# kije/gpu_raytracer

Hardware: AMD Instinct MI355X
Metric: Mrays/s (higher is better)
Workload: dtype f32

## Files before the change

gpu_raytracer_amd/api.py:

```python
import ctypes as C
import os
import sys

import numpy as np

from . import types as T

_HERE = os.path.dirname(os.path.abspath(__file__))
LIB_PATH = os.environ.get("RT_HIP_LIB", os.path.join(_HERE, "librt_hip.so"))

RT_OK = 0
ERRORS = {-1: "RT_ERR_BAD_ARG", -2: "RT_ERR_OOM", -3: "RT_ERR_HIP", -4: "RT_ERR_NOT_UPLOADED", -5: "RT_ERR_INTERNAL"}
MODE_LEGACY, MODE_WAVEFRONT, MODE_EXTENDED = 0, 1, 2
FLAG_COUNTERS = 1
FLAG_NO_SHADOWS = 2
FLAG_KERNEL_V1 = 4
FLAG_KERNEL_SM = 8
FLAG_NO_SHADOW_GRID = 16
FLAG_KERNEL_PIPELINE = 32
FLAG_NO_BEAMS = 64
FLAG_STAGE_TIMES = 128
FLAG_ACCUMULATE = 256
FLAG_ACCUMULATE_RESTART = 512
ACCUMULATE_MAX_SAMPLES = 1 << 24
PREPARE_SHADOW_GRIDS = 1
PREPARE_QUALITY_TREE = 2
QUERY_COUNTERS = 1
QUERY_CHUNK = 4194304
QUERY_COUNT_ALL = 2
MULTI_HIT_MAX = 16
AO_MAX_SAMPLES = 4096
DIRECT_AMBIENT, DIRECT_NO_SHADOWS, DIRECT_NO_SHADOW_GRID = 4, 8, 16
DIRECT_MAX_LIGHTS = 32
PATH_NO_SHADOWS, PATH_CAMERA_DRAWS = 32, 64
PATH_MAX_SAMPLES = 4096
MAX_BOUNCES = T.MAX_BOUNCES
UPDATE_REBUILD = 1
AOV_SAMPLES_PER_LAUNCH = T.AOV_SAMPLES_PER_LAUNCH
DENOISE_DEMODULATE = T.DENOISE_DEMODULATE
DENOISE_MAX_ITERATIONS = T.DENOISE_MAX_ITERATIONS
DENOISE_DEFAULTS = dict(iterations=T.DENOISE_DEFAULT_ITERATIONS, sigma_color=T.DENOISE_DEFAULT_SIGMA_COLOR, sigma_normal=T.DENOISE_DEFAULT_SIGMA_NORMAL,
                        sigma_depth=T.DENOISE_DEFAULT_SIGMA_DEPTH, sigma_albedo=T.DENOISE_DEFAULT_SIGMA_ALBEDO)
STAT_MEGAKERNEL_FALLBACK, STAT_SINGLE_PASS, STAT_REFIT, STAT_REBUILT = 1, 2, 4, 8
PRIM_MISS = 0xFFFFFFFF
PRIM_SPHERE_FLAG = 0x80000000
EXTENDED_AVAILABLE = True

ABI_SYMBOLS = [
    "rt_create", "rt_upload_scene", "rt_upload_scene_packed", "rt_upload_textures", "rt_prepare", "rt_render", "rt_dispatch_tile",
    "rt_read_rgb32f", "rt_read_rgba8_channels", "rt_read_rgba8_combined", "rt_read_hits",
    "rt_get_stats", "rt_last_error", "rt_destroy", "rt_version",
    "rt_intersect", "rt_occluded", "rt_camera_rays", "rt_intersect_all",
    "rt_surface", "rt_ambient_occlusion", "rt_direct_light", "rt_radiance", "rt_closest_point",
    "rt_update_geometry",
    "rt_accumulated_samples",
    "rt_aovs", "rt_sample_rays", "rt_denoise",
    "rt_render_adaptive", "rt_read_adaptive",
]


class RtError(RuntimeError):
    def __init__(self, code, msg):
        super().__init__(f"{ERRORS.get(code, code)}: {msg}")
        self.code = code


_lib = None


def load():
    global _lib
    if _lib is None:
        if not os.path.exists(LIB_PATH):
            raise ImportError(f"{LIB_PATH} is missing: build it with `python -m gpu_raytracer_amd.build` "
                              "(there is no CPU fallback for the hot path)")
        lib = C.CDLL(LIB_PATH)
        lib.rt_last_error.restype = C.c_char_p
        lib.rt_last_error.argtypes = [C.c_void_p]
        lib.rt_version.restype = C.c_char_p
        lib.rt_destroy.restype = None
        lib.rt_destroy.argtypes = [C.c_void_p]
        for name in ABI_SYMBOLS:
            if "RT_HIP_LIB" in os.environ and not hasattr(lib, name):
                continue
            fn = getattr(lib, name)
            if name not in ("rt_last_error", "rt_version", "rt_destroy"):
                fn.restype = C.c_int
        _lib = lib
    return _lib


def _p(a):
    return C.c_void_p(a.ctypes.data) if a is not None and a.size else C.c_void_p(0)



def _is_torch(x):
    return type(x).__module__.split(".")[0] == "torch"


def _check_batch(a, name, cols, dtype_name):
    if _is_torch(a):
        import torch
        want = {"float32": torch.float32, "bool": torch.bool}[dtype_name]
        if a.dtype != want:
            raise TypeError(f"{name}: dtype {a.dtype}, expected torch.{dtype_name}")
        shape, contiguous = tuple(a.shape), a.is_contiguous()
    elif isinstance(a, np.ndarray):
        if a.dtype != np.dtype(dtype_name):
            raise TypeError(f"{name}: dtype {a.dtype}, expected {dtype_name}")
        shape, contiguous = a.shape, a.flags.c_contiguous
    else:
        raise TypeError(f"{name}: a numpy array or a torch tensor, not {type(a).__name__}")
    if (cols and (len(shape) != 2 or shape[1] != cols)) or (not cols and len(shape) != 1):
        raise ValueError(f"{name}: shape {shape}, expected {'(N, %d)' % cols if cols else '(N,)'}")
    if not contiguous:
        raise ValueError(f"{name}: not C-contiguous")
    return shape[0]


def _contiguous(a):
    return a.is_contiguous() if _is_torch(a) else a.flags.c_contiguous


def _check_kind_dtype(a, name, dtype_name):
    if _is_torch(a):
        import torch
        if a.dtype != getattr(torch, dtype_name):
            raise TypeError(f"{name}: dtype {a.dtype}, expected torch.{dtype_name}")
    elif not isinstance(a, np.ndarray):
        raise TypeError(f"{name}: a numpy array or a torch tensor, not {type(a).__name__}")
    elif a.dtype != np.dtype(dtype_name):
        raise TypeError(f"{name}: dtype {a.dtype}, expected {dtype_name}")


def _check_hit_lists(a, n, max_hits):
    _check_kind_dtype(a, "out", "float32")
    if len(a.shape) != 3 or tuple(a.shape[1:]) != (max_hits, 4):
        raise ValueError(f"out: shape {tuple(a.shape)}, expected (N, {max_hits}, 4)")
    if not _contiguous(a):
# ... 237 lines not shown
        self._check(self.lib.rt_prepare(self._h, C.c_uint32(what)))

    def render(self, width, height, camera, mode=MODE_LEGACY, spp=1, max_bounces=4, frame_seed=0, tile_size=0,
               tile_rank=0, tile_world=1, counters=False, no_shadows=False, kernel_v1=False, kernel_sm=False, no_shadow_grid=False, kernel_pipeline=False, no_beams=False, stage_times=False,
               accumulate=False, restart=False):
        p = render_params(width, height, camera, mode=mode, spp=spp, max_bounces=max_bounces, frame_seed=frame_seed, tile_size=tile_size,
                          tile_rank=tile_rank, tile_world=tile_world, counters=counters, no_shadows=no_shadows, kernel_v1=kernel_v1,
                          kernel_sm=kernel_sm, no_shadow_grid=no_shadow_grid, kernel_pipeline=kernel_pipeline, no_beams=no_beams,
                          stage_times=stage_times, accumulate=accumulate, restart=restart)
        self._check(self.lib.rt_render(self._h, _p(p)))
        self.width, self.height = width, height
        return self.stats()

    def accumulated_samples(self):
        n = C.c_uint32(0)
        self._check(self.lib.rt_accumulated_samples(self._h, C.byref(n)))
        return n.value

    def render_adaptive(self, width, height, camera, spp, threshold, min_samples=4, restart=False, **render_kw):
        render_kw.setdefault("mode", MODE_EXTENDED)
        p = render_params(width, height, camera, spp=spp, accumulate=True, restart=restart, **render_kw)
        ap = np.zeros((), dtype=T.ADAPTIVE_PARAMS)
        ap["threshold"], ap["min_samples"] = threshold, min_samples
        self._check(self.lib.rt_render_adaptive(self._h, _p(p), _p(ap)))
        self.width, self.height = width, height
        return self.stats()

    def read_adaptive(self):
        out = np.zeros((self.height, self.width, 8), np.float32)
        self._check(self.lib.rt_read_adaptive(self._h, _p(out), C.c_size_t(self.height * self.width)))
        return out

    def dispatch_tile(self, pc):
        pcb = np.ascontiguousarray(pc)
        self._check(self.lib.rt_dispatch_tile(self._h, _p(pcb)))
        res = pcb["resolution"].reshape(-1)
        self.width, self.height = int(res[0]), int(res[1])

    def read_rgb32f(self):
        out = np.zeros((self.height, self.width, 3), np.float32)
        self._check(self.lib.rt_read_rgb32f(self._h, _p(out), C.c_size_t(out.size)))
        return out

    def read_rgba8_channels(self):
        outs = [np.zeros((self.height, self.width, 4), np.uint8) for _ in range(3)]
        self._check(self.lib.rt_read_rgba8_channels(self._h, _p(outs[0]), _p(outs[1]), _p(outs[2]), C.c_size_t(outs[0].size)))
        return outs

    def read_rgba8_combined(self):
        out = np.zeros((self.height, self.width, 4), np.uint8)
        self._check(self.lib.rt_read_rgba8_combined(self._h, _p(out), C.c_size_t(out.size)))
        return out

    def read_hits(self):
        prim = np.zeros((self.height, self.width), np.uint32)
        t = np.zeros((self.height, self.width), np.float32)
        self._check(self.lib.rt_read_hits(self._h, _p(prim), _p(t), C.c_size_t(prim.size)))
        return prim, t

    def debug_beams(self, n_blocks):
        out = np.zeros(n_blocks, np.uint32)
        m = self.lib.rt_debug_beams(self._h, _p(out), C.c_uint32(n_blocks))
        if m < 0:
            raise RtError(m, "rt_debug_beams")
        return out[:m]

    def debug_stage_times(self):
        out = (C.c_double * 2)()
        self._check(self.lib.rt_debug_stage_times(self._h, out))
        return float(out[0]), int(out[1])

    def debug_counters(self):
        out = (C.c_ulonglong * 8)()
        self._check(self.lib.rt_debug_counters(self._h, out))
        names = ("transition_passes", "transition_lanes", "node_iters", "node_lanes", "leaf_iters", "leaf_lanes", "cycles_transition", "cycles_traversal")
        return dict(zip(names, [int(v) for v in out]))

    def debug_shadow_grid(self, light=None):
        out = (C.c_ulonglong * 8)()
        self._check(self.lib.rt_debug_shadow_grid(self._h, C.c_uint32(0xFFFFFFFF if light is None else light), out))
        names = ("lights_with_grid", "entries", "bytes", "segments_answered", "entries_read") if light is None else ("kind", "res", "entries", "near", "longest", "heavy_cells", "filled_cells")
        return dict(zip(names, [int(v) for v in out]))

    def debug_check_bvh(self):
        out = (C.c_uint32 * 8)()
        fails = self.lib.rt_debug_check_bvh(self._h, out)
        names = ("nodes", "leaves", "depth", "real_depth", "placed_once", "method", "nodes_hash", "tris_hash")
        d = dict(zip(names, [int(v) for v in out]))
        d["failures"] = int(fails)
        return d

    def _query(self, fn, rays, out, cols, dtype_name, counters, in_cols=8, in_name="rays"):
        n = _check_batch(rays, in_name, in_cols, "float32")
        shape = (n, cols) if cols else (n,)
        if out is None:
            out = _empty_like_batch(rays, shape, dtype_name)
        else:
            if _is_torch(out) != _is_torch(rays):
                raise TypeError(f"out: must be the same kind (numpy / torch) as {in_name}")
            if _check_batch(out, "out", cols, dtype_name) != n:
                raise ValueError(f"out: {len(out)} rows for {n} {in_name}")
        _sync_torch(rays, out)
        self._check(getattr(self.lib, fn)(self._h, _addr(rays), C.c_size_t(n), _addr(out), C.c_uint32(QUERY_COUNTERS if counters else 0)))
        return out

    def intersect(self, rays, out=None, counters=False):
        return self._query("rt_intersect", rays, out, 4, "float32", counters)

    def occluded(self, rays, out=None, counters=False):
        return self._query("rt_occluded", rays, out, 0, "bool", counters)

    def intersect_all(self, rays, max_hits, out=None, counts=None, count_all=False, counters=False):
        n = _check_batch(rays, "rays", 8, "float32")
        if isinstance(max_hits, bool) or not isinstance(max_hits, (int, np.integer)) or not 0 <= max_hits <= MULTI_HIT_MAX:
            raise ValueError(f"max_hits: {max_hits!r}, expected an integer in 0 .. {MULTI_HIT_MAX}")
        max_hits = int(max_hits)
        if max_hits == 0 and not count_all:
            raise ValueError("max_hits: 0 lists nothing, which needs count_all=True (a pure crossing count)")
        torch_kind = _is_torch(rays)
        for name, a in (("out", out), ("counts", counts)):
            if a is not None and _is_torch(a) != torch_kind:
                raise TypeError(f"{name}: must be the same kind (numpy / torch) as rays")
        if max_hits == 0:
            out = None
        elif out is None:
            out = _empty_like_batch(rays, (n, max_hits, 4), "float32")
        else:
            _check_hit_lists(out, n, max_hits)
        if counts is None:
            if torch_kind:
                import torch
                counts = torch.empty((n,), dtype=torch.int32, device=rays.device)
            else:
                counts = np.empty((n,), np.uint32)
        else:
            _check_counts(counts, n)
        _sync_torch(rays, out, counts)
        flags = (QUERY_COUNTERS if counters else 0) | (QUERY_COUNT_ALL if count_all else 0)
        self._check(self.lib.rt_intersect_all(self._h, _addr(rays), C.c_size_t(n), C.c_uint32(max_hits),
                                              _addr(out) if out is not None else C.c_void_p(0), _addr(counts), C.c_uint32(flags)))
        return out, counts

    def surface(self, rays, out=None, counters=False):
        return self._query("rt_surface", rays, out, 8, "float32", counters)

    def ambient_occlusion(self, points, samples, seed=0, max_distance=float("inf"), bias=1e-3, out=None, counts=None, counters=False):
        n = _check_batch(points, "points", 8, "float32")
        if isinstance(samples, bool) or not isinstance(samples, (int, np.integer)) or not 1 <= samples <= AO_MAX_SAMPLES:
            raise ValueError(f"samples: {samples!r}, expected an integer in 1 .. {AO_MAX_SAMPLES}")
        if isinstance(seed, bool) or not isinstance(seed, (int, np.integer)) or not 0 <= seed <= 0xFFFFFFFF:
            raise ValueError(f"seed: {seed!r}, expected an integer in 0 .. 2^32 - 1")
        try:
            max_distance, bias = float(max_distance), float(bias)
        except (TypeError, ValueError):
            raise ValueError(f"max_distance / bias: {max_distance!r}, {bias!r}, expected numbers") from None
        if not max_distance > 0:
            raise ValueError(f"max_distance: {max_distance!r}, expected > 0 (inf allowed)")
        if not (np.isfinite(bias) and bias >= 0):
            raise ValueError(f"bias: {bias!r}, expected finite and >= 0")
        torch_kind = _is_torch(points)
        for name, a in (("out", out), ("counts", counts)):
            if a is not None and _is_torch(a) != torch_kind:
                raise TypeError(f"{name}: must be the same kind (numpy / torch) as points")
        if out is None:
            out = _empty_like_batch(points, (n,), "float32")
        elif _check_batch(out, "out", 0, "float32") != n:
            raise ValueError(f"out: {out.shape[0]} rows for {n} points")
        if counts is None:
            if torch_kind:
                import torch
                counts = torch.empty((n,), dtype=torch.int32, device=points.device)
            else:
                counts = np.empty((n,), np.uint32)
        else:
            _check_counts(counts, n, "points")
        ap = np.zeros((), dtype=T.AO_PARAMS)
        ap["samples"], ap["seed"], ap["max_distance"], ap["bias"] = int(samples), int(seed), max_distance, bias
        ap["flags"] = QUERY_COUNTERS if counters else 0
        _sync_torch(points, out, counts)
        self._check(self.lib.rt_ambient_occlusion(self._h, _addr(points), C.c_size_t(n), _p(ap), _addr(out), _addr(counts)))
        return out, counts

    def direct_light(self, points, bias=1e-3, ambient=False, shadows=True, use_grids=True, out=None, counters=False):
        n = _check_batch(points, "points", 8, "float32")
        try:
            bias = float(bias)
        except (TypeError, ValueError):
            raise ValueError(f"bias: {bias!r}, expected a number") from None
        if not (np.isfinite(bias) and bias >= 0):
            raise ValueError(f"bias: {bias!r}, expected finite and >= 0")
        if out is None:
            out = _empty_like_batch(points, (n, 4), "float32")
        else:
            if _is_torch(out) != _is_torch(points):
                raise TypeError("out: must be the same kind (numpy / torch) as points")
            if _check_batch(out, "out", 4, "float32") != n:
                raise ValueError(f"out: {out.shape[0]} rows for {n} points")
        dp = np.zeros((), dtype=T.DIRECT_LIGHT_PARAMS)
        dp["bias"] = bias
        dp["flags"] = ((DIRECT_AMBIENT if ambient else 0) | (0 if shadows else DIRECT_NO_SHADOWS) | (0 if use_grids else DIRECT_NO_SHADOW_GRID)
                       | (QUERY_COUNTERS if counters else 0))
        _sync_torch(points, out)
        self._check(self.lib.rt_direct_light(self._h, _addr(points), C.c_size_t(n), _p(dp), _addr(out)))
        return out

    def radiance(self, rays, samples=1, max_bounces=4, seed=0, first_sample=0, shadows=True, camera_draws=False, out=None, counters=False):
        n = _check_batch(rays, "rays", 8, "float32")
        for name, v, lo, hi in (("samples", samples, 1, PATH_MAX_SAMPLES), ("max_bounces", max_bounces, 0, MAX_BOUNCES), ("seed", seed, 0, 0xFFFFFFFF),
                                ("first_sample", first_sample, 0, 0xFFFFFFFF)):
            if isinstance(v, bool) or not isinstance(v, (int, np.integer)) or not lo <= v <= hi:
                raise ValueError(f"{name}: {v!r}, expected an integer in {lo} .. {hi}")
        if int(first_sample) + int(samples) > 1 << 32:
            raise ValueError(f"first_sample: {first_sample!r} + samples {samples!r} passes 2^32")
        if out is None:
            out = _empty_like_batch(rays, (n, 4), "float32")
        else:
            if _is_torch(out) != _is_torch(rays):
                raise TypeError("out: must be the same kind (numpy / torch) as rays")
            if _check_batch(out, "out", 4, "float32") != n:
                raise ValueError(f"out: {out.shape[0]} rows for {n} rays")
        pp = np.zeros((), dtype=T.PATH_PARAMS)
        pp["samples"], pp["max_bounces"], pp["seed"], pp["first_sample"] = int(samples), int(max_bounces), int(seed), int(first_sample)
        pp["flags"] = (0 if shadows else PATH_NO_SHADOWS) | (PATH_CAMERA_DRAWS if camera_draws else 0) | (QUERY_COUNTERS if counters else 0)
        _sync_torch(rays, out)
        self._check(self.lib.rt_radiance(self._h, _addr(rays), C.c_size_t(n), _p(pp), _addr(out)))
        return out

    def closest_point(self, points, out=None, counters=False):
        return self._query("rt_closest_point", points, out, 8, "float32", counters, in_cols=4, in_name="points")

    def camera_rays(self, width, height, camera, mode=MODE_LEGACY, out=None):
        cam = np.zeros((), T.CAMERA)
        cam[...] = camera
        n = width * height
        if out is None:
            out = np.empty((n, 8), np.float32)
        elif _check_batch(out, "out", 8, "float32") != n:
            raise ValueError(f"out: {len(out)} rows for {n} pixels")
        _sync_torch(out)
        self._check(self.lib.rt_camera_rays(self._h, _p(cam), C.c_uint32(width), C.c_uint32(height), C.c_uint32(mode), _addr(out)))
        return out

    def aovs(self, width, height, camera, out=None, **render_kw):
        p = render_params(width, height, camera, **render_kw)
        if out is None:
            out = np.empty((height, width, 8), np.float32)
        else:
            _check_image(out, "out", height, width, 8)
        _sync_torch(out)
        self._check(self.lib.rt_aovs(self._h, _p(p), _addr(out)))
        return out

    def sample_rays(self, width, height, camera, sample, out=None, **render_kw):
        render_kw.setdefault("mode", MODE_EXTENDED)
        p = render_params(width, height, camera, **render_kw)
        n = width * height
        if out is None:
            out = np.empty((n, 8), np.float32)
        elif _check_batch(out, "out", 8, "float32") != n:
            raise ValueError(f"out: {len(out)} rows for {n} pixels")
        _sync_torch(out)
        self._check(self.lib.rt_sample_rays(self._h, _p(p), C.c_uint32(sample), _addr(out)))
        return out

    def denoise(self, rgb, aovs, out=None, iterations=DENOISE_DEFAULTS["iterations"], sigma_color=DENOISE_DEFAULTS["sigma_color"],
                sigma_normal=DENOISE_DEFAULTS["sigma_normal"], sigma_depth=DENOISE_DEFAULTS["sigma_depth"],
                sigma_albedo=DENOISE_DEFAULTS["sigma_albedo"], demodulate=True):
        if _is_torch(rgb) != _is_torch(aovs):
            raise TypeError("aovs: must be the same kind (numpy / torch) as rgb")
        h, w = (tuple(getattr(rgb, "shape", ())) + (0, 0))[:2]
        _check_image(rgb, "rgb", h, w, 3)
        _check_image(aovs, "aovs", h, w, 8)
        if out is None:
            out = _empty_like_batch(rgb, (h, w, 3), "float32")
        else:
            if _is_torch(out) != _is_torch(rgb):
                raise TypeError("out: must be the same kind (numpy / torch) as rgb")
            _check_image(out, "out", h, w, 3)
        dp = np.zeros((), dtype=T.DENOISE_PARAMS)
        dp["width"], dp["height"], dp["iterations"] = w, h, iterations
        dp["flags"] = DENOISE_DEMODULATE if demodulate else 0
        dp["sigma_color"], dp["sigma_normal"], dp["sigma_depth"], dp["sigma_albedo"] = sigma_color, sigma_normal, sigma_depth, sigma_albedo
        _sync_torch(rgb, aovs, out)
        self._check(self.lib.rt_denoise(self._h, _p(dp), _addr(rgb), _addr(aovs), _addr(out)))
# ... 11 lines not shown
```

gpu_raytracer_amd/csrc/direct_light.h:

```cpp
#ifndef RT_DIRECT_LIGHT_H
#define RT_DIRECT_LIGHT_H

#include <hip/hip_runtime.h>

#include "device_layout.h"
#include "shadow_grid.h"

namespace rt {

struct DirectLightArgs {
    float bias;
    uint32_t ambient, shadows;
    const DevShadowGrid* grids;
    float lo[3], hi[3];
};

inline void direct_light_box(const float box_lo[3], const float box_hi[3], float lo[3], float hi[3]) {
    float m = 0.0f;
    for (int a = 0; a < 3; a++) m = box_hi[a] - box_lo[a] > m ? box_hi[a] - box_lo[a] : m;
    for (int a = 0; a < 3; a++) lo[a] = box_lo[a] - m, hi[a] = box_hi[a] + m;
}

#define RT_CNT_DL_GRID_ANSWERED 6u
#define RT_CNT_DL_GRID_ENTRIES 7u
hipError_t launch_direct_light(const DevScene& sc, const DirectLightArgs& a, const void* points, void* out, uint32_t n, bool count,
                               unsigned long long* counters, hipStream_t stream);

}
#endif
```

gpu_raytracer_amd/csrc/direct_light.hip:

```cpp
#include "direct_light.h"

#include "device_common.h"
#include "shadow_grid_walk.h"

using namespace rtdev;

namespace {

__device__ __forceinline__ bool finite3(V3 a) { return isfinite(a.x) && isfinite(a.y) && isfinite(a.z); }

__device__ __forceinline__ bool segment_valid(V3 o, V3 d, float dist) {
    return finite3(o) && finite3(d) && !(d.x == 0.0f && d.y == 0.0f && d.z == 0.0f) && RT_MIN_RAY_DISTANCE < dist;
}

#ifndef RT_DL_MIN_WAVES
#define RT_DL_MIN_WAVES 6
#endif
template <bool COUNT>
__global__ __launch_bounds__(WAVE, COUNT ? RT_DL_MIN_WAVES - 2 : RT_DL_MIN_WAVES) void k_dl_direct(DevScene sc, rt::DirectLightArgs a, const float4* __restrict__ points, uint4* __restrict__ out,
                                                     uint32_t n, unsigned long long* __restrict__ counters) {
    extern __shared__ uint2 s_stack[];
    __shared__ uint32_t s_upto[WAVE], s_occ[WAVE];
    const uint32_t lane = threadIdx.x;
    uint2* stack = s_stack + lane;
    DevLight* s_lights = reinterpret_cast<DevLight*>(s_stack + (size_t)(sc.stack_entries / 2u + 1u) * WAVE);
    DevShadowGrid* s_grids = reinterpret_cast<DevShadowGrid*>(s_lights + sc.n_lights);
    stage_lights(s_lights, sc);
    if (a.grids) {
        const uint32_t words = sc.n_lights * (uint32_t)(sizeof(DevShadowGrid) / 4);
        const uint32_t* __restrict__ src = reinterpret_cast<const uint32_t*>(a.grids);
        uint32_t* dst = reinterpret_cast<uint32_t*>(s_grids);
        for (uint32_t k = lane; k < words; k += WAVE) dst[k] = src[k];
        __syncthreads();
    }
    const uint32_t i = blockIdx.x * WAVE + lane;
    float4 pa = make_float4(0.0f, 0.0f, 0.0f, 0.0f), pb = pa;
    if (i < n) {
        pa = points[2 * (size_t)i], pb = points[2 * (size_t)i + 1];
        RT_KEEP4(pa);
        RT_KEEP4(pb);
    }
    const V3 P = v3(pa.x, pa.y, pa.z), N = v3(pb.x, pb.y, pb.z);
    const uint32_t material_id = __float_as_uint(pb.w);
    const bool is_point = i < n && finite3(P) && finite3(N) && !(N.x == 0.0f && N.y == 0.0f && N.z == 0.0f);
    const bool shade = is_point && material_id < sc.n_materials;
    DevMaterial m = {};
    if (shade) m = sc.materials[material_id];
    const bool shadows = a.shadows != 0u;
    const bool eligible = a.grids != nullptr && shade && fabsf(dot(N, N) - 1.0f) <= 1.0e-5f && P.x >= a.lo[0] && P.x <= a.hi[0] && P.y >= a.lo[1] &&
                          P.y <= a.hi[1] && P.z >= a.lo[2] && P.z <= a.hi[2];
    const V3 o = P + N * a.bias;
    uint32_t nonzero = 0, occ = 0, walk = 0;
    uint32_t n_tests = 0, n_entries = 0, n_answered = 0;
    Counts cnt = {0u, 0u};
    for (uint32_t li = 0; li < sc.n_lights; li++) {
        V3 sdir = v3(0.0f, 0.0f, 0.0f);
        float sdist = 0.0f;
        bool nz = false;
        if (shade) nz = needs_shadow_segment(light_contribution(s_lights[li], m, P, N, sdir, sdist));
        if (nz) nonzero |= 1u << li;
        const bool mine = nz && shadows;
        if (!eligible) {
            if (mine) walk |= 1u << li;
            continue;
        }
        if (__ballot(mine) == 0ull) continue;
        if (mine && segment_valid(o, sdir, sdist)) {
            GridPending pd = {};
            uint32_t outcome = grid_segment_head<COUNT>(sc, s_lights[li], s_grids[li], P, N, pd, n_tests, n_entries);
            if (outcome == GRID_PENDING) outcome = grid_walk_on<COUNT>(s_grids[li], pd, RT_WF_GRID_WALK, n_tests, n_entries);
            if (COUNT && outcome <= GRID_OCCLUDED) n_answered++;
            if (outcome == GRID_OCCLUDED) occ |= 1u << li;
            if (outcome >= GRID_FORWARD) walk |= 1u << li;
        }
    }
    {
        uint32_t upto = (uint32_t)__popc(walk);
        for (uint32_t off = 1; off < WAVE; off <<= 1) {
            const uint32_t t = __shfl_up(upto, off, WAVE);
            if (lane >= off) upto += t;
        }
        const uint32_t total = __shfl(upto, WAVE - 1, WAVE);
        if (total) {
            s_upto[lane] = upto;
            s_occ[lane] = 0u;
            __syncthreads();
            for (uint32_t first = 0; first < total; first += WAVE) {
                const uint32_t s = first + lane;
                uint32_t src = 0;
                for (uint32_t step = WAVE / 2; step; step >>= 1)
                    if (s_upto[src + step - 1u] <= s) src += step;
                uint32_t rest = __shfl(walk, src, WAVE);
                const V3 sp = v3(__shfl(P.x, src, WAVE), __shfl(P.y, src, WAVE), __shfl(P.z, src, WAVE));
                const V3 so = v3(__shfl(o.x, src, WAVE), __shfl(o.y, src, WAVE), __shfl(o.z, src, WAVE));
                if (s < total) {
                    for (uint32_t k = s - (src ? s_upto[src - 1u] : 0u); k; k--) rest &= rest - 1u;
                    const uint32_t li = (uint32_t)__ffs(rest) - 1u;
                    V3 sdir;
                    float sdist;
                    shadow_segment(s_lights[li], sp, sdir, sdist);
                    if (segment_valid(so, sdir, sdist) && occluded<COUNT>(sc, so, sdir, RT_MIN_RAY_DISTANCE, sdist, stack, cnt)) atomicOr(&s_occ[src], 1u << li);
                }
            }
            __syncthreads();
            occ |= s_occ[lane];
        }
    }
    uint4 r = make_uint4(0u, 0u, 0u, 0u);
    if (shade) {
        const V3 rad = ext_light_sum(s_lights, sc.n_lights, m, P, N, a.ambient != 0u, shadows, [&](uint32_t li, V3, float) { return ((occ >> li) & 1u) == 0u; });
        r = make_uint4(__float_as_uint(rad.x), __float_as_uint(rad.y), __float_as_uint(rad.z), nonzero & ~occ);
    } else if (is_point) {
        const V3 c = RT_MAGENTA();
        r = make_uint4(__float_as_uint(c.x), __float_as_uint(c.y), __float_as_uint(c.z), 0u);
    }
    if (i < n) out[i] = r;
    const unsigned long long segments = wave_sum(shadows ? (uint32_t)__popc(nonzero) : 0u);
    if (lane == 0 && segments) atomicAdd(&counters[RT_CNT_SHADOW], segments);
    if (COUNT) {
        const unsigned long long n0 = wave_sum(cnt.nodes), n1 = wave_sum(cnt.tris + n_tests), ga = wave_sum(n_answered), ge = wave_sum(n_entries);
        if (lane == 0) {
            atomicAdd(&counters[RT_CNT_NODE_VISITS], n0);
            atomicAdd(&counters[RT_CNT_TRI_TESTS], n1);
            atomicAdd(&counters[RT_CNT_DL_GRID_ANSWERED], ga);
            atomicAdd(&counters[RT_CNT_DL_GRID_ENTRIES], ge);
        }
    }
}

}

namespace rt {

hipError_t launch_direct_light(const DevScene& sc, const DirectLightArgs& a, const void* points, void* out, uint32_t n, bool count,
                               unsigned long long* counters, hipStream_t stream) {
    if (n == 0) return hipSuccess;
    const dim3 grid((n + WAVE - 1) / WAVE), block(WAVE);
    const size_t lds = (size_t)(sc.stack_entries / 2u + 1u) * WAVE * sizeof(uint2)
                       + (size_t)sc.n_lights * (sizeof(DevLight) + (a.grids ? sizeof(DevShadowGrid) : 0));
    const float4* p = reinterpret_cast<const float4*>(points);
    uint4* o = reinterpret_cast<uint4*>(out);
    if (count) hipLaunchKernelGGL((k_dl_direct<true>), grid, block, lds, stream, sc, a, p, o, n, counters);
    else hipLaunchKernelGGL((k_dl_direct<false>), grid, block, lds, stream, sc, a, p, o, n, counters);
    return hipGetLastError();
}

}
```

gpu_raytracer_amd/csrc/rt_context.cpp:

```cpp
#include "rt_internal.h"

#include "bvh_check.h"

namespace rti {
namespace { thread_local std::string g_create_error; }

int sync_pending(rt_ctx* ctx) {
    if (!ctx->pending_dispatch) return RT_OK;
    ctx->pending_dispatch = false;
    DeviceState& d = ctx->devs[0];
    HIPCHK(ctx, hipSetDevice(d.device));
    HIPCHK(ctx, hipStreamSynchronize(d.stream));
    float ms = 0.0f;
    HIPCHK(ctx, hipEventElapsedTime(&ms, d.ev0, d.ev1));
    ctx->stats.kernel_ms = ms;
    return RT_OK;
}

}

using namespace rti;

extern "C" {

// ... 80 lines not shown
    std::vector<uint32_t> seen(ctx->n_input_tris, 0);
    uint32_t real_depth = 0;
    size_t leaves = 0;
    rtcheck::g_print = true;
    int fails = rtcheck::check_tree(b, seen, &real_depth, &leaves);
    uint32_t once = 0;
    for (uint32_t v : seen) {
        once += v == 1 ? 1u : 0u;
        if (v > 1) fails++;
    }
    if (out) {
        out[0] = (uint32_t)b.nodes.size();
        out[1] = (uint32_t)leaves;
        out[2] = b.depth;
        out[3] = real_depth;
        out[4] = once;
        out[5] = ctx->stats.tree_build;
        out[6] = rtcheck::hash_nodes(b);
        out[7] = rtcheck::hash_tris(b);
    }
    return fails;
}

unsigned long long rt_debug_queue_slots(unsigned long long max_entries, uint32_t per_lane, unsigned long long waves) {
    return rt::wf_queue_slots_for((size_t)max_entries, per_lane, (size_t)waves);
}
uint32_t rt_debug_pick_window(uint32_t iterations, uint32_t per_lane) { return rt::wf_pick_window(iterations, per_lane); }
unsigned long long rt_debug_state_slots(unsigned long long paths, unsigned long long waves) { return rt::wf_state_slots_for((size_t)paths, (size_t)waves); }

int rt_debug_beams(rt_ctx* ctx, uint32_t* counts, uint32_t n) {
    if (!ctx || ctx->devs.empty()) return RT_ERR_BAD_ARG;
    DeviceState& d = ctx->devs[0];
    if (!d.pipe.wf.beam_count) return 0;
    if (hipSetDevice(d.device) != hipSuccess) return RT_ERR_HIP;
    (void)hipStreamSynchronize(d.stream);
    const uint32_t m = std::min(n, d.pipe.wf.n_blocks);
    if (m && hipMemcpy(counts, d.pipe.wf.beam_count, (size_t)m * 4, hipMemcpyDeviceToHost) != hipSuccess) return RT_ERR_HIP;
    for (uint32_t i = 0; i < m; i++)
        if (counts[i] & RT_BEAM_OVERFLOW) counts[i] = 0xFFFFFFFFu;
    return (int)m;
}

int rt_debug_stage_times(rt_ctx* ctx, double out[2]) {
    if (!ctx || !out) return RT_ERR_BAD_ARG;
    out[0] = ctx->stage_ms[0];
    out[1] = ctx->stage_ms[1];
    return RT_OK;
}

int rt_debug_counters(rt_ctx* ctx, unsigned long long out[8]) {
    if (!ctx || !out) return RT_ERR_BAD_ARG;
    for (int k = 0; k < 8; k++) out[k] = ctx->diag[k];
    return RT_OK;
}

int rt_debug_shadow_grid(rt_ctx* ctx, uint32_t light, unsigned long long out[8]) {
    if (!ctx || !out) return RT_ERR_BAD_ARG;
    for (int k = 0; k < 8; k++) out[k] = 0;
    if (ctx->devs.empty()) return RT_OK;
    const DeviceState& d = ctx->devs[0];
    if (light == 0xFFFFFFFFu) {
        for (const rt::ShadowGridBuild& g : d.grids.info) {
            if (g.grid.kind == RT_SG_KIND_NONE) continue;
            out[0]++;
            out[1] += g.n_entries;
            out[2] += g.bytes;
        }
        out[3] = ctx->grid_diag[0];
        out[4] = ctx->grid_diag[1];
        return RT_OK;
    }
    if (light >= d.grids.info.size()) return RT_OK;
    const rt::ShadowGridBuild& g = d.grids.info[light];
    out[0] = g.grid.kind;
    out[1] = g.grid.res;
    out[2] = g.n_entries;
    out[3] = g.near_count;
    out[4] = g.longest;
    out[5] = g.heavy_cells;
    out[6] = g.filled_cells;
    return RT_OK;
}

int rt_get_stats(rt_ctx* ctx, rt_stats* out) {
    if (!ctx) return RT_ERR_BAD_ARG;
    if (!out) return ctx->fail(RT_ERR_BAD_ARG, "rt_get_stats: null out");
    if (int rcp = sync_pending(ctx)) return rcp;
    *out = ctx->stats;
    return RT_OK;
}

}
```

gpu_raytracer_amd/csrc/rt_frame.cpp:

```cpp
#include "rt_internal.h"

#ifndef RT_SINGLE_PASS_MAX_NODES
#define RT_SINGLE_PASS_MAX_NODES 64u
#endif
#ifndef RT_WF_LANES_DEFAULT
#define RT_WF_LANES_DEFAULT 2
#endif

namespace rti {
DevCamera make_camera(const rt_camera& cam, float res_x, float res_y, bool wavefront) {
    DevCamera c;
    float wf, hf;
    if (wavefront) {
        wf = res_x;
        hf = res_y;
    } else {
        auto as_u32 = [](float f) -> uint32_t { return !(f > 0.0f) ? 0u : (f >= 4294967296.0f ? 0xFFFFFFFFu : (uint32_t)f); };
        wf = (float)as_u32(res_x);
        hf = (float)as_u32(res_y);
    }
    c.width_f = wf;
    c.height_f = hf;
    c.aspect = wf / hf;
    c.fov_scale = tanf(cam.fov * 0.5f * 3.14159265358979323846f / 180.0f);
// ... 235 lines not shown
    if (two_lanes && n_batches > 1 && (n_batches & 1u)) {
        const uint32_t fewer = n_batches - 1, b = (spp + fewer - 1) / fewer;
        if ((uint64_t)b * per_sample * 10 <= target_paths * 11 && b <= hard_limit && (uint64_t)b * per_sample <= free_bytes / 2 / bytes_per_path) n_batches = fewer;
        else n_batches++;
    }
    return std::max(1u, (spp + n_batches - 1) / std::max(1u, n_batches));
}

uint32_t single_pass_max_nodes() {
    if (const char* e = std::getenv("RT_SINGLE_PASS_MAX_NODES")) return (uint32_t)std::strtoul(e, nullptr, 10);
    return RT_SINGLE_PASS_MAX_NODES;
}

void assign_tiles(DevFrame& f, DeviceState& d, uint32_t world, uint32_t rank, size_t nd, size_t j) {
    frame_share(f, world, rank, nd, j);
    d.tile_first = f.tile_first;
    d.tile_stride = f.tile_stride;
    d.n_owned = f.n_owned_tiles;
}

struct KernelChoice {
    rt::FrameKernel kernel;
    bool fallback;
};

KernelChoice choose_kernel(const rt_ctx* ctx, const DevFrame& f) {
    using rt::FrameKernel;
    const DevScene& sc = ctx->scene_counts;
    if (f.mode != RT_MODE_EXTENDED) return {FrameKernel::REFERENCE, false};
    if (f.flags & RT_FLAG_KERNEL_V1) return {FrameKernel::MEGAKERNEL_V1, false};
    if (f.flags & RT_FLAG_KERNEL_SM) return {FrameKernel::MEGAKERNEL_SM, false};
    if (!(f.flags & RT_FLAG_KERNEL_PIPELINE) && f.max_bounce == 0 && sc.n_nodes <= single_pass_max_nodes()) return {FrameKernel::SINGLE_PASS, false};
    const bool fits = sc.n_lights <= RT_WF_MAX_LIGHTS && (uint64_t)f.n_owned_tiles * rt::blocks_per_tile(f.tile_size) * 64u <= wavefront_max_paths(sc.n_lights);
    return fits ? KernelChoice{FrameKernel::PIPELINE, false} : KernelChoice{FrameKernel::MEGAKERNEL_SM, true};
}

struct WfRun {
    enum Phase { GENERATE, BOUNCE, RESOLVE, DONE };
    Phase phase = DONE;
    bool pipeline = false;
    size_t dev = 0;
    DevFrame f{};
    DevScene dsc{};
    uint32_t batch = 1, first = 0, j = 0, it = 0, alive = 0;
    uint32_t n_blocks = 0;
    bool two = false;
    bool beams = false;
    hipStream_t poll_stream = nullptr;
};

int setup_pipeline(rt_ctx* ctx, size_t j, const DevFrame& f, WfRun& r) {
    DeviceState& d = ctx->devs[j];
    const uint32_t n_lights = ctx->scene_counts.n_lights;
    if (!(f.flags & (RT_FLAG_NO_SHADOW_GRID | RT_FLAG_NO_SHADOWS)))
        if (int rc = ensure_grids(ctx, d)) return rc;
    const uint32_t n_blocks = f.adaptive ? d.ad.live_blocks : f.n_owned_tiles * rt::blocks_per_tile(f.tile_size);
    size_t free_b = 0, total_b = 0;
    HIPCHK(ctx, hipMemGetInfo(&free_b, &total_b));
    const char* lanes_env = std::getenv("RT_WF_LANES");
    bool two_lanes_on = lanes_env ? std::atoi(lanes_env) >= 2 : (RT_WF_LANES_DEFAULT >= 2 && d.grids.table.get() != nullptr && !(f.flags & RT_FLAG_NO_SHADOW_GRID));
    if (!lanes_env && two_lanes_on && f.max_bounce > 4 && wavefront_batch(n_blocks, f.spp, n_lights, free_b, false) >= f.spp) two_lanes_on = false;
    const uint32_t batch = d.pipe.wf.n_blocks == n_blocks && d.wf_spp == f.spp && d.pipe.wf.batch && d.pipe.lights >= n_lights && d.used_two_lanes == (two_lanes_on && f.spp >= 2) ? d.pipe.wf.batch
                                                                                               : wavefront_batch(n_blocks, f.spp, n_lights, two_lanes_on ? free_b / 2 : free_b, two_lanes_on);
    d.wf_spp = f.spp;
    const uint32_t n_batches = (f.spp + batch - 1) / batch;
    const bool two = two_lanes_on && n_batches >= 2 && d.stream2;
    if (int rc = ensure_wavefront(ctx, d, n_blocks, batch, n_lights, two, f.adaptive != 0)) return rc;
    HIPCHK(ctx, hipMemsetAsync(d.pipe.wf.totals, 0, rt::WF_N_TOTALS * sizeof(unsigned long long), d.stream));
    if (!f.adaptive) HIPCHK(ctx, hipEventRecord(d.ev0, d.stream));
    const char* be = std::getenv("RT_WF_BEAMS");
    const bool beams = !(f.flags & RT_FLAG_NO_BEAMS) && (be ? std::atoi(be) != 0 : true);
    if (beams) {
        rt::WfBuffers wb = d.pipe.wf;
        wb.n_blocks = n_blocks;
        wb.batch = batch;
        HIPCHK(ctx, rt::wf_beams(scene_for(ctx, d), f, wb, d.stream));
    }
    if (two) {
        HIPCHK(ctx, hipEventRecord(d.ev_start, d.stream));
        HIPCHK(ctx, hipStreamWaitEvent(d.stream2, d.ev_start, 0));
        HIPCHK(ctx, hipMemsetAsync(d.pipe.wf2.totals, 0, rt::WF_N_TOTALS * sizeof(unsigned long long), d.stream2));
    }
    d.pipe.wf.grids = d.pipe.wf2.grids = (f.flags & RT_FLAG_NO_SHADOW_GRID) ? nullptr : d.grids.table.get();
    const char* pe = std::getenv("RT_WF_PROBE");
    d.pipe.wf.probe = d.pipe.wf2.probe = pe ? (uint32_t)std::atoi(pe) : 0u;
    d.used_two_lanes = two;
    r = WfRun{};
    r.phase = WfRun::GENERATE;
    r.pipeline = true;
    r.dev = j;
    r.f = f;
    r.dsc = scene_for(ctx, d);
    r.batch = batch;
    r.n_blocks = n_blocks;
    r.two = two;
    r.beams = beams;
    return RT_OK;
}

struct WfLane { rt::WfBuffers w; hipStream_t st; };
WfLane lane_of(const DeviceState& d, const WfRun& r) {
    const bool second = r.two && (r.j & 1u);
    WfLane l{second ? d.pipe.wf2 : d.pipe.wf, second ? d.stream2 : d.stream};
    if (!r.beams) l.w.beam_count = nullptr;
    l.w.n_blocks = r.n_blocks;
    l.w.batch = r.batch;
    return l;
}
uint32_t batch_samples(const WfRun& r) { return std::min(r.batch, r.f.spp - r.first); }

int wf_step_generate(rt_ctx* ctx, DeviceState& d, WfRun& r, const WfLane& l) {
    HIPCHK(ctx, rt::wf_generate(r.dsc, r.f, l.w, targets_for(d, r.f), r.first, batch_samples(r), l.st));
    r.it = 0;
    r.phase = WfRun::BOUNCE;
    return RT_OK;
}

int wf_step_bounce(rt_ctx* ctx, DeviceState& d, WfRun& r, const WfLane& l, bool counters, std::vector<WfRun*>& polls) {
    hipEvent_t* gev = nullptr;
    if ((r.f.flags & RT_FLAG_STAGE_TIMES) && r.dev == 0 && rt::wf_runs_shadow_grid(r.f, l.w)) {
        if (d.stage_events.size() < (size_t)d.stage_events_used + 2) {
            hipEvent_t a = nullptr, b = nullptr;
            HIPCHK(ctx, hipEventCreate(&a));
            HIPCHK(ctx, hipEventCreate(&b));
            d.stage_events.push_back(a);
            d.stage_events.push_back(b);
        }
        gev = d.stage_events.data() + d.stage_events_used;
        d.stage_events_used += 2;
    }
    HIPCHK(ctx, rt::wf_bounce(r.dsc, r.f, l.w, r.it, batch_samples(r), counters, l.st, gev));
    if (r.it >= r.f.max_bounce) r.phase = WfRun::RESOLVE;
    else if ((r.it & 7u) == 7u) {
        HIPCHK(ctx, hipMemcpyAsync(&r.alive, l.w.counters + rt::WF_EXT_COUNT, 4, hipMemcpyDeviceToHost, l.st));
        r.poll_stream = l.st;
        polls.push_back(&r);
    } else r.it++;
    return RT_OK;
}

int wf_step_resolve(rt_ctx* ctx, DeviceState& d, WfRun& r, const WfLane& l) {
    const uint32_t n = batch_samples(r);
    if (r.two && r.j > 0) HIPCHK(ctx, hipStreamWaitEvent(l.st, d.ev_res[(r.j - 1u) & 1u], 0));
    HIPCHK(ctx, rt::wf_resolve(r.f, l.w, targets_for(d, r.f), n, r.first, r.first == 0, r.first + n >= r.f.spp, l.st));
    if (r.two) HIPCHK(ctx, hipEventRecord(d.ev_res[r.j & 1u], l.st));
    r.first += r.batch;
    r.j++;
    if (r.first < r.f.spp) {
        r.phase = WfRun::GENERATE;
        return RT_OK;
    }
    if (r.two) {
        HIPCHK(ctx, hipEventRecord(d.ev_join, d.stream2));
        HIPCHK(ctx, hipStreamWaitEvent(d.stream, d.ev_join, 0));
    }
    if (r.f.adaptive) HIPCHK(ctx, rt::launch_ad_image(r.f, targets_for(d, r.f), d.stream));
    HIPCHK(ctx, hipEventRecord(d.ev1, d.stream));
    r.phase = WfRun::DONE;
    return RT_OK;
}

struct FrameTotals {
    double kernel_ms = 0.0;
    uint64_t pixels = 0;
    unsigned long long segments = 0, camera = 0, continuation = 0, shadow = 0, node_visits = 0, tri_tests = 0;
    unsigned long long diag[RT_CNT_N_DIAG] = {0};
    unsigned long long grid_answered = 0, grid_entries = 0;
};

void add_counters(FrameTotals& t, const unsigned long long (&c)[RT_CNT_SLOTS]) {
    t.segments += c[RT_CNT_SEGMENTS], t.camera += c[RT_CNT_CAMERA], t.continuation += c[RT_CNT_CONTINUATION], t.shadow += c[RT_CNT_SHADOW];
    t.node_visits += c[RT_CNT_NODE_VISITS], t.tri_tests += c[RT_CNT_TRI_TESTS];
    for (int k = 0; k < RT_CNT_N_DIAG; k++) t.diag[k] += c[RT_CNT_DIAG + k];
}

void merge_lanes(unsigned long long (&t)[rt::WF_N_TOTALS], const unsigned long long (&t2)[rt::WF_N_TOTALS]) {
    for (int k = 0; k < rt::WF_N_TOTALS; k++) t[k] = k == rt::WF_TOTAL_STACK_MAX ? std::max(t[k], t2[k]) : t[k] + t2[k];
}

int add_totals(rt_ctx* ctx, FrameTotals& t, const unsigned long long (&w)[rt::WF_N_TOTALS]) {
    t.segments += w[rt::WF_TOTAL_CAMERA] + w[rt::WF_TOTAL_CONTINUATION] + w[rt::WF_TOTAL_SHADOW];
    t.camera += w[rt::WF_TOTAL_CAMERA], t.continuation += w[rt::WF_TOTAL_CONTINUATION], t.shadow += w[rt::WF_TOTAL_SHADOW];
    t.node_visits += w[rt::WF_TOTAL_NODE_VISITS], t.tri_tests += w[rt::WF_TOTAL_TRI_TESTS];
    if (w[rt::WF_TOTAL_ERROR] != 0)
        return ctx->fail(RT_ERR_INTERNAL, "wavefront pipeline: %s (frame discarded)",
                         (w[rt::WF_TOTAL_ERROR] & 2ull) ? "a traversal stack grew beyond the depth the tree reports" : "a queue reservation exceeded its allocation");
    t.diag[0] = std::max(t.diag[0], w[rt::WF_TOTAL_STACK_MAX]);
    for (int k = 1; k < RT_CNT_N_DIAG; k++) t.diag[k] += w[rt::WF_TOTAL_STACK_MAX + k];
    t.grid_answered += w[rt::WF_TOTAL_GRID_ANSWERED], t.grid_entries += w[rt::WF_TOTAL_GRID_ENTRIES];
    return RT_OK;
}

uint64_t share_pixels(const DevFrame& fr, const DeviceState& d) {
    if (fr.single_tile)
        return (uint64_t)std::min(fr.tile_w, fr.width - std::min(fr.width, fr.tile_off_x)) * std::min(fr.tile_h, fr.height - std::min(fr.height, fr.tile_off_y));
    return owned_pixels(fr, d.tile_first, d.tile_stride, d.n_owned);
}

int collect_device(rt_ctx* ctx, size_t j, const DevFrame& fr, bool counters, const WfRun& r, FrameTotals& t) {
    DeviceState& d = ctx->devs[j];
    HIPCHK(ctx, hipSetDevice(d.device));
    HIPCHK(ctx, hipStreamSynchronize(d.stream));
    float ms = 0.0f;
    HIPCHK(ctx, hipEventElapsedTime(&ms, d.ev0, d.ev1));
    t.kernel_ms = std::max(t.kernel_ms, (double)ms);
    if (j == 0 && d.stage_events_used) {
        if (d.stream2) HIPCHK(ctx, hipStreamSynchronize(d.stream2));
        for (uint32_t k = 0; k + 1 < d.stage_events_used; k += 2) {
            float sm = 0.0f;
            HIPCHK(ctx, hipEventElapsedTime(&sm, d.stage_events[k], d.stage_events[k + 1]));
            ctx->stage_ms[0] += sm;
            ctx->stage_ms[1] += 1.0;
        }
    }
    if (r.pipeline) {
        unsigned long long w[rt::WF_N_TOTALS];
        HIPCHK(ctx, hipMemcpy(w, d.pipe.wf.totals, sizeof w, hipMemcpyDeviceToHost));
        if (r.two) {
            unsigned long long w2[rt::WF_N_TOTALS];
            HIPCHK(ctx, hipMemcpy(w2, d.pipe.wf2.totals, sizeof w2, hipMemcpyDeviceToHost));
            merge_lanes(w, w2);
        }
        if (int rc = add_totals(ctx, t, w)) return rc;
    } else if (counters || fr.mode == RT_MODE_EXTENDED) {
        unsigned long long c[RT_CNT_SLOTS];
        HIPCHK(ctx, hipMemcpy(c, d.counters.get(), sizeof c, hipMemcpyDeviceToHost));
        add_counters(t, c);
    }
    t.pixels += fr.adaptive ? d.ad.pixels : share_pixels(fr, d);
    return RT_OK;
}

void finish_frame(rt_ctx* ctx, const DevFrame& fr, bool counters, const FrameTotals& t, uint32_t stat_flags, double w0) {
    rt_stats& st = ctx->stats;
    st.pixels = t.pixels;
    if (fr.mode == RT_MODE_EXTENDED) {
        st.rays = t.segments, st.primary_rays = t.camera, st.continuation_rays = t.continuation, st.shadow_rays = t.shadow;
    } else {
        const bool traced = fr.mode == RT_MODE_LEGACY || fr.cur_bounce <= fr.max_bounce;
        st.rays = traced ? t.pixels : 0;
        st.primary_rays = st.rays;
        st.continuation_rays = st.shadow_rays = 0;
    }
    st.node_visits = counters ? t.node_visits : 0;
    st.tri_tests = counters ? t.tri_tests : 0;
    for (int k = 0; k < RT_CNT_N_DIAG; k++) ctx->diag[k] = counters ? t.diag[k] : 0;
    ctx->grid_diag[0] = counters ? t.grid_answered : 0, ctx->grid_diag[1] = counters ? t.grid_entries : 0;
    st.kernel_ms = t.kernel_ms, st.wall_ms = now_ms() - w0, st.flags = stat_flags;
}

int run_frame(rt_ctx* ctx, DevFrame fr, bool counters, uint32_t world, uint32_t rank, bool single_tile) {
    const double w0 = now_ms();
    if (!single_tile || counters)
        if (int rc = sync_pending(ctx)) return rc;
    const size_t nd = single_tile ? 1 : ctx->devs.size();
    std::vector<WfRun> runs(nd);
    uint32_t stat_flags = 0;
    for (size_t j = 0; j < nd; j++) ctx->devs[j].stage_events_used = 0;
    ctx->stage_ms[0] = ctx->stage_ms[1] = 0.0;
    for (size_t j = 0; j < nd; j++) {
        DeviceState& d = ctx->devs[j];
        HIPCHK(ctx, hipSetDevice(d.device));
        if (int rc = ensure_targets(ctx, d, fr.width, fr.height)) return rc;
        DevFrame f = fr;
        if (!single_tile) assign_tiles(f, d, world, rank, nd, j);
        HIPCHK(ctx, hipMemsetAsync(d.counters.get(), 0, RT_CNT_SLOTS * sizeof(unsigned long long), d.stream));
        HIPCHK(ctx, hipEventRecord(d.ev0, d.stream));
        if (f.adaptive) {
            f.ad_mask = d.ad.mask.get();
            f.ad_blocks = d.ad.blocks.get();
            unsigned long long counts[2] = {0, 0};
            HIPCHK(ctx, rt::launch_ad_select(f, targets_for(d, f), d.ad.mask.get(), d.ad.blocks.get(), d.ad.counts.get(), d.stream));
            HIPCHK(ctx, hipMemcpyAsync(counts, d.ad.counts.get(), sizeof counts, hipMemcpyDeviceToHost, d.stream));
            HIPCHK(ctx, hipStreamSynchronize(d.stream));
            d.ad.live_blocks = (uint32_t)counts[0];
            d.ad.pixels = counts[1];
            if (d.ad.live_blocks == 0) {
                HIPCHK(ctx, rt::launch_ad_image(f, targets_for(d, f), d.stream));
                HIPCHK(ctx, hipEventRecord(d.ev1, d.stream));
                continue;
            }
        }
        const KernelChoice k = choose_kernel(ctx, f);
        stat_flags |= (k.fallback ? RT_STAT_MEGAKERNEL_FALLBACK : 0u) | (k.kernel == rt::FrameKernel::SINGLE_PASS ? RT_STAT_SINGLE_PASS : 0u);
        if (k.kernel == rt::FrameKernel::PIPELINE) {
            if (int rc = setup_pipeline(ctx, j, f, runs[j])) return rc;
            continue;
        }
        if (k.kernel == rt::FrameKernel::REFERENCE) HIPCHK(ctx, rt::launch_render_reference(scene_for(ctx, d), f, targets_for(d, f), counters, d.stream));
        else HIPCHK(ctx, rt::launch_render_extended(scene_for(ctx, d), f, targets_for(d, f), k.kernel, counters, d.stream));
        if (f.adaptive) HIPCHK(ctx, rt::launch_ad_image(f, targets_for(d, f), d.stream));
        HIPCHK(ctx, hipEventRecord(d.ev1, d.stream));
    }
    for (bool busy = true; busy;) {
        busy = false;
        std::vector<WfRun*> polls;
        for (WfRun& r : runs) {
            if (r.phase == WfRun::DONE) continue;
            busy = true;
            DeviceState& d = ctx->devs[r.dev];
            HIPCHK(ctx, hipSetDevice(d.device));
            const WfLane l = lane_of(d, r);
            const int rc = r.phase == WfRun::GENERATE ? wf_step_generate(ctx, d, r, l) : r.phase == WfRun::BOUNCE ? wf_step_bounce(ctx, d, r, l, counters, polls) : wf_step_resolve(ctx, d, r, l);
            if (rc != RT_OK) return rc;
        }
        for (WfRun* r : polls) {
            HIPCHK(ctx, hipSetDevice(ctx->devs[r->dev].device));
            HIPCHK(ctx, hipStreamSynchronize(r->poll_stream));
            if (r->alive == 0) r->phase = WfRun::RESOLVE;
            else r->it++;
        }
    }
    if (single_tile && !counters && fr.mode != RT_MODE_EXTENDED) {
        rt_stats& st = ctx->stats;
        st.pixels = share_pixels(fr, ctx->devs[0]);
        st.rays = st.primary_rays = (fr.mode == RT_MODE_LEGACY || fr.cur_bounce <= fr.max_bounce) ? st.pixels : 0;
        st.continuation_rays = st.shadow_rays = st.node_visits = st.tri_tests = 0;
        st.kernel_ms = 0.0;
        st.wall_ms = now_ms() - w0;
        ctx->pending_dispatch = true;
        return RT_OK;
    }
    FrameTotals t;
    for (size_t j = 0; j < nd; j++)
        if (int rc = collect_device(ctx, j, fr, counters, runs[j], t)) return rc;
    finish_frame(ctx, fr, counters, t, stat_flags, w0);
    return RT_OK;
}

int accumulation_of(rt_ctx* ctx, const char* fn, const rt_render_params* p, uint32_t world, uint32_t rank, bool adaptive, DevFrame& fr, AccumKey& key) {
// ... 127 lines not shown
```

gpu_raytracer_amd/csrc/rt_internal.h:

```cpp
#ifndef RT_INTERNAL_H
#define RT_INTERNAL_H

#include <hip/hip_runtime.h>

#include <algorithm>
#include <chrono>
#include <cmath>
#include <cstdarg>
#include <cstdio>
#include <cstdlib>
#include <cstring>
#include <string>
#include <utility>
#include <vector>

#include "../../include/rt_hip.h"
#include "adaptive.h"
#include "bvh_builder.h"
#include "closest_point.h"
#include "denoise.h"
#include "device_build.h"
#include "device_layout.h"
#include "direct_light.h"
#include "half.h"
#include "kernels.h"
#include "path_query.h"
#include "ray_query.h"
#include "refit.h"
#include "shadow_grid.h"
#include "surface_query.h"
#include "wavefront.h"

#define HIPCHK(ctx, call)                                                                                       \
    do {                                                                                                        \
        hipError_t e_ = (call);                                                                                 \
        if (e_ != hipSuccess)                                                                                   \
            return (ctx)->fail(e_ == hipErrorOutOfMemory ? RT_ERR_OOM : RT_ERR_HIP, "%s failed: %s (%s:%d)", #call, \
                               hipGetErrorString(e_), __FILE__, __LINE__);                                     \
    } while (0)

namespace rti __attribute__((visibility("hidden"))) {

template <bool Pinned>
class Mem {
    void* p_ = nullptr;
    size_t bytes_ = 0;
public:
    Mem() = default;
    Mem(void* adopted, size_t bytes) : p_(adopted), bytes_(adopted ? bytes : 0) {}
    Mem(Mem&& o) noexcept : p_(std::exchange(o.p_, nullptr)), bytes_(std::exchange(o.bytes_, 0)) {}
    Mem& operator=(Mem&& o) noexcept {
        if (this != &o) reset(), p_ = std::exchange(o.p_, nullptr), bytes_ = std::exchange(o.bytes_, 0);
        return *this;
    }
    ~Mem() { reset(); }
    void reset() {
        if (p_) (void)(Pinned ? hipHostFree(p_) : hipFree(p_));
        p_ = nullptr, bytes_ = 0;
    }
    hipError_t reserve(size_t bytes) {
        if (bytes_ >= bytes) return hipSuccess;
        reset();
        const hipError_t e = Pinned ? hipHostMalloc(&p_, bytes, hipHostMallocDefault) : hipMalloc(&p_, bytes);
        if (e != hipSuccess) p_ = nullptr;
        else bytes_ = bytes;
        return e;
    }
    void* get() const { return p_; }
};
using DevMem = Mem<false>;
using PinnedMem = Mem<true>;
template <class T>
struct DevBuf : DevMem {
    using DevMem::DevMem;
    T* get() const { return static_cast<T*>(DevMem::get()); }
};

struct DeviceState {
    int device = -1;
    hipStream_t stream = nullptr;
    hipStream_t stream2 = nullptr;
    hipEvent_t ev0 = nullptr, ev1 = nullptr;
    hipEvent_t ev_start = nullptr, ev_join = nullptr, ev_res[2] = {nullptr, nullptr};
    std::vector<hipEvent_t> stage_events;
    uint32_t stage_events_used = 0;
    std::vector<hipEvent_t> rq_events;
    DevBuf<unsigned long long> counters;
    uint32_t tile_first = 0, tile_stride = 1, n_owned = 0;

    struct Scene {
        DevBuf<DevNode8> nodes;
        DevBuf<DevTri> tris;
        DevBuf<DevSphere> spheres;
        DevBuf<DevLight> lights;
        DevBuf<DevMaterial> materials;
        DevBuf<float> verts;
    } scene;
    struct Grids {
        DevBuf<DevShadowGrid> table;
        std::vector<DevMem> allocs;
        std::vector<rt::ShadowGridBuild> info;
        bool tried = false;
    } grids;
    struct Refit {
        DevBuf<uint32_t> vidx;
        DevBuf<uint32_t> order;
        DevBuf<float4> boxes;
        DevBuf<uint32_t> dropped;
        DevBuf<uint32_t> flag;
    } refit;
    struct Targets {
        DevBuf<float> rgba32f;
        DevBuf<uint8_t> chan[3];
        DevBuf<uint32_t> prim_id;
        DevBuf<float> hit_t;
        uint32_t w = 0, h = 0;
        DevMem readback_dev;
        PinnedMem readback_host;
    } fb;
    struct Lanes {
        rt::WfBuffers wf{};
        rt::WfBuffers wf2{};
        std::vector<DevMem> allocs, allocs2;
        uint32_t lights = 0;
    } pipe;
    bool used_two_lanes = false;
    uint32_t wf_spp = 0;
    struct Query {
        DevMem in, out, counts;
        DevBuf<uint32_t> ao;
        DevBuf<uint4> paths;
    } rq;
    struct Accum {
        DevBuf<float> run_sum, run_odd;
        uint32_t w = 0, h = 0;
    } acc;
    struct Adaptive {
        DevBuf<unsigned long long> mask;
        DevBuf<uint32_t> blocks;
        DevBuf<unsigned long long> counts;
        uint32_t cap = 0, live_blocks = 0;
        uint64_t pixels = 0;
    } ad;
    struct Denoise {
        DevMem aov, rgb;
        DevBuf<float4> plane[2];
    } dn;
};

struct AccumKey {
    rt_camera camera;
    uint32_t width, height, max_bounces, frame_seed, tile_size, tile_rank, tile_world, no_shadows;
    uint32_t adaptive;
};

}

struct rt_ctx {
    std::vector<rti::DeviceState> devs;
    std::string err;
    bool uploaded = false;
    bool pending_dispatch = false;
    DevScene scene_counts{};
    rt_stats stats{};
    uint32_t frame_w = 0, frame_h = 0, frame_tile = RT_TILE_SIZE, frame_tiles_x = 0, frame_tiles_y = 0;
    bool frame_valid = false;
    unsigned long long diag[RT_CNT_N_DIAG] = {0};
    unsigned long long grid_diag[2] = {0};
    double stage_ms[2] = {0.0, 0.0};
    int fail_upload_at = -1;
    uint32_t n_input_tris = 0;
    std::vector<rt::BuildTri> build_tris;
    std::vector<DevLight> host_lights;
    float box_lo[3] = {0, 0, 0}, box_hi[3] = {0, 0, 0};
    std::vector<rt_triangle> up_triangles;
    std::vector<uint32_t> up_prim_ids;
    uint32_t up_vertices = 0;
    bool rf_ready = false;
    std::vector<uint32_t> rf_level_first;
    uint32_t rf_n_dropped = 0;
    bool host_geometry_stale = false;
    uint32_t n_textures = 0;
    uint64_t texture_bytes = 0;
    rti::AccumKey acc_key{};
    uint32_t acc_samples = 0;

    int fail(int code, const char* fmt, ...) {
        char buf[512];
        va_list ap;
        va_start(ap, fmt);
        vsnprintf(buf, sizeof buf, fmt, ap);
        va_end(ap);
        err = buf;
        return code;
    }
};

namespace rti __attribute__((visibility("hidden"))) {

inline double now_ms() { return std::chrono::duration<double, std::milli>(std::chrono::steady_clock::now().time_since_epoch()).count(); }

inline void end_accumulation(rt_ctx* ctx) { ctx->acc_samples = 0; }

struct QueryPtr {
    bool device = false;
    size_t dev = 0;
};

int sync_pending(rt_ctx* ctx);
void free_scene(DeviceState& d);
int ensure_grids(rt_ctx* ctx, DeviceState& d);
DevCamera make_camera(const rt_camera& cam, float res_x, float res_y, bool wavefront);
DevScene scene_for(const rt_ctx* ctx, const DeviceState& d);
void frame_share(DevFrame& f, uint32_t world, uint32_t rank, size_t nd, size_t j);
uint64_t owned_pixels(const DevFrame& fr, uint32_t first, uint32_t stride, uint32_t n_owned);
int frame_of_params(rt_ctx* ctx, const char* fn, const rt_render_params* p, DevFrame& fr, uint32_t& world, uint32_t& rank);
void copy_share(uint8_t* dst, const uint8_t* src, size_t elem, uint32_t w, uint32_t h, uint32_t ts, uint32_t tiles_x, uint32_t first, uint32_t stride,
                uint32_t n_owned);
int consolidate_on_first_device(rt_ctx* ctx, uint32_t w, uint32_t h);
int classify_ptr(rt_ctx* ctx, const char* fn, const char* what, const void* p, QueryPtr& q, uintptr_t align = 16);

}
#endif
```

gpu_raytracer_amd/csrc/rt_query.cpp:

```cpp
#include "rt_internal.h"

namespace rti {
int classify_ptr(rt_ctx* ctx, const char* fn, const char* what, const void* p, QueryPtr& q, uintptr_t align) {
    q = QueryPtr{};
    hipPointerAttribute_t a{};
    if (hipPointerGetAttributes(&a, p) != hipSuccess) {
        (void)hipGetLastError();
        return RT_OK;
    }
    if (a.type != hipMemoryTypeDevice || a.isManaged) return RT_OK;
    for (size_t j = 0; j < ctx->devs.size(); j++)
        if (ctx->devs[j].device == a.device) {
            if (reinterpret_cast<uintptr_t>(p) & (align - 1))
                return ctx->fail(RT_ERR_BAD_ARG, "%s: %s is device memory that is not %u-byte aligned (%p)", fn, what, (unsigned)align, p);
            q.device = true;
            q.dev = j;
            return RT_OK;
        }
    return ctx->fail(RT_ERR_BAD_ARG, "%s: %s is device memory of HIP device %d, which is not a device of this context", fn, what, a.device);
}

namespace {

int ensure_query_events(rt_ctx* ctx, DeviceState& d, size_t n) {
// ... 177 lines not shown
        for (size_t j = 0; j < nd; j++) first[j] = n * j / nd, count[j] = n * (j + 1) / nd - first[j];
    auto enqueue = [&](size_t j) -> int {
        DeviceState& d = ctx->devs[j];
        HIPCHK(ctx, hipSetDevice(d.device));
        const DevScene sc = scene_for(ctx, d);
        const size_t chunks = (count[j] + chunk - 1) / chunk;
        if (int rc = ensure_query_events(ctx, d, 2 * chunks)) return rc;
        const size_t most = std::min<size_t>(count[j], chunk);
        HIPCHK(ctx, d.rq.ao.reserve(most * sizeof(uint32_t)));
        if (!pin.device) {
            HIPCHK(ctx, d.rq.in.reserve(most * sizeof(rt_surface_point)));
            if (visibility) HIPCHK(ctx, d.rq.out.reserve(most * sizeof(float)));
        }
        if (counters) HIPCHK(ctx, hipMemsetAsync(d.counters.get(), 0, (RT_CNT_TRI_TESTS + 1) * sizeof(unsigned long long), d.stream));
        for (size_t c = 0; c < chunks; c++) {
            const size_t off = first[j] + c * chunk, m = std::min<size_t>(chunk, first[j] + count[j] - off);
            const void* in = points + off;
            float* vis = visibility ? visibility + off : nullptr;
            uint32_t* cnt_out = unoccluded ? unoccluded + off : nullptr;
            if (!pin.device) {
                HIPCHK(ctx, hipMemcpyAsync(d.rq.in.get(), in, m * sizeof(rt_surface_point), hipMemcpyHostToDevice, d.stream));
                in = d.rq.in.get();
                vis = visibility ? static_cast<float*>(d.rq.out.get()) : nullptr;
                cnt_out = nullptr;
            }
            HIPCHK(ctx, hipEventRecord(d.rq_events[2 * c], d.stream));
            HIPCHK(ctx, hipMemsetAsync(d.rq.ao.get(), 0, m * sizeof(uint32_t), d.stream));
            HIPCHK(ctx, rt::launch_ao(sc, in, off, (uint32_t)m, ap, d.rq.ao.get(), counters ? d.counters.get() : nullptr, d.stream));
            if (vis || cnt_out) HIPCHK(ctx, rt::launch_ao_finish(d.rq.ao.get(), (uint32_t)m, ap.samples, vis, cnt_out, d.stream));
            HIPCHK(ctx, hipEventRecord(d.rq_events[2 * c + 1], d.stream));
            if (!pin.device && visibility) HIPCHK(ctx, hipMemcpyAsync(visibility + off, vis, m * sizeof(float), hipMemcpyDeviceToHost, d.stream));
            if (!pin.device && unoccluded) HIPCHK(ctx, hipMemcpyAsync(unoccluded + off, d.rq.ao.get(), m * sizeof(uint32_t), hipMemcpyDeviceToHost, d.stream));
        }
        return RT_OK;
    };
    for (size_t j = 0; j < nd; j++)
        if (count[j] > 0)
            if (int rc = enqueue(j)) {
                drain_streams(ctx);
                return rc;
            }
    double kernel_ms = 0.0;
    unsigned long long nodes = 0, tris = 0;
    for (size_t j = 0; j < nd; j++) {
        if (count[j] == 0) continue;
        DeviceState& d = ctx->devs[j];
        hipError_t e = hipSetDevice(d.device);
        if (e == hipSuccess) e = hipStreamSynchronize(d.stream);
        if (e != hipSuccess) {
            drain_streams(ctx);
            return ctx->fail(RT_ERR_HIP, "%s: device %d: %s", fn, d.device, hipGetErrorString(e));
        }
        double ms = 0.0;
        for (size_t c = 0; c * chunk < count[j]; c++) {
            float cm = 0.0f;
            HIPCHK(ctx, hipEventElapsedTime(&cm, d.rq_events[2 * c], d.rq_events[2 * c + 1]));
            ms += cm;
        }
        kernel_ms = std::max(kernel_ms, ms);
        if (counters) {
            unsigned long long cn[RT_CNT_TRI_TESTS + 1];
            HIPCHK(ctx, hipMemcpy(cn, d.counters.get(), sizeof cn, hipMemcpyDeviceToHost));
            nodes += cn[RT_CNT_NODE_VISITS];
            tris += cn[RT_CNT_TRI_TESTS];
        }
    }
    rt_stats& st = ctx->stats;
    st.rays = (uint64_t)n * p->samples;
    st.primary_rays = st.continuation_rays = st.shadow_rays = st.pixels = 0;
    st.node_visits = counters ? nodes : 0;
    st.tri_tests = counters ? tris : 0;
    st.kernel_ms = kernel_ms;
    st.wall_ms = now_ms() - w0;
    return RT_OK;
}

static_assert(RT_DIRECT_MAX_LIGHTS == RT_WF_MAX_LIGHTS, "the grid table and lit_mask hold one entry / bit per light, as the pipeline's visibility word");
int run_direct_light(rt_ctx* ctx, const rt_surface_point* points, size_t n, const rt_direct_light_params* p, rt_lighting* out) {
    const char* fn = "rt_direct_light";
    const double w0 = now_ms();
    if (!ctx) return RT_ERR_BAD_ARG;
    if (n == 0) return RT_OK;
    if (!points || !p || !out) return ctx->fail(RT_ERR_BAD_ARG, "%s: %s is NULL with n = %zu", fn, !points ? "points" : !p ? "params" : "out", n);
    const uint32_t known = RT_QUERY_COUNTERS | RT_DIRECT_AMBIENT | RT_DIRECT_NO_SHADOWS | RT_DIRECT_NO_SHADOW_GRID;
    if (p->flags & ~known) return ctx->fail(RT_ERR_BAD_ARG, "%s: unknown flag bits 0x%x", fn, p->flags & ~known);
    if (!std::isfinite(p->bias) || p->bias < 0.0f) return ctx->fail(RT_ERR_BAD_ARG, "%s: bias %g (finite and >= 0)", fn, (double)p->bias);
    if (!ctx->uploaded) return ctx->fail(RT_ERR_NOT_UPLOADED, "%s: no scene uploaded", fn);
    if (ctx->scene_counts.n_lights > RT_DIRECT_MAX_LIGHTS)
        return ctx->fail(RT_ERR_BAD_ARG, "%s: the scene has %u lights (at most %u: one bit of lit_mask each)", fn, ctx->scene_counts.n_lights, RT_DIRECT_MAX_LIGHTS);
    if (int rcp = sync_pending(ctx)) return rcp;
    QueryPtr pin, pout;
    if (int rc = classify_ptr(ctx, fn, "points", points, pin)) return rc;
    if (int rc = classify_ptr(ctx, fn, "out", out, pout)) return rc;
    if (pin.device != pout.device || pin.dev != pout.dev)
        return ctx->fail(RT_ERR_BAD_ARG, "%s: points and out must both be host memory or both device memory of the same device", fn);
    rt::DirectLightArgs args{};
    args.bias = p->bias;
    args.ambient = (p->flags & RT_DIRECT_AMBIENT) ? 1u : 0u;
    args.shadows = (p->flags & RT_DIRECT_NO_SHADOWS) ? 0u : 1u;
    const float grid_bias = RT_SG_EXT_EPS;
    const bool grids_allowed = args.shadows && !(p->flags & RT_DIRECT_NO_SHADOW_GRID) && std::memcmp(&p->bias, &grid_bias, sizeof(float)) == 0;
    rt::direct_light_box(ctx->box_lo, ctx->box_hi, args.lo, args.hi);
    const size_t chunk = RT_QUERY_CHUNK;
    const bool counters = (p->flags & RT_QUERY_COUNTERS) != 0;
    const size_t nd = ctx->devs.size();
    std::vector<size_t> first(nd, 0), count(nd, 0);
    if (pin.device) count[pin.dev] = n;
    else
        for (size_t j = 0; j < nd; j++) first[j] = n * j / nd, count[j] = n * (j + 1) / nd - first[j];
    auto enqueue = [&](size_t j) -> int {
        DeviceState& d = ctx->devs[j];
        HIPCHK(ctx, hipSetDevice(d.device));
        const DevScene sc = scene_for(ctx, d);
        rt::DirectLightArgs a = args;
        a.grids = grids_allowed ? d.grids.table.get() : nullptr;
        const size_t chunks = (count[j] + chunk - 1) / chunk;
        if (int rc = ensure_query_events(ctx, d, 2 * chunks)) return rc;
        if (!pin.device) {
            const size_t most = std::min<size_t>(count[j], chunk);
            HIPCHK(ctx, d.rq.in.reserve(most * sizeof(rt_surface_point)));
            HIPCHK(ctx, d.rq.out.reserve(most * sizeof(rt_lighting)));
        }
        HIPCHK(ctx, hipMemsetAsync(d.counters.get(), 0, RT_CNT_DIAG * sizeof(unsigned long long), d.stream));
        for (size_t c = 0; c < chunks; c++) {
            const size_t off = first[j] + c * chunk, m = std::min<size_t>(chunk, first[j] + count[j] - off);
            const void* in = points + off;
            void* res = out + off;
            if (!pin.device) {
                HIPCHK(ctx, hipMemcpyAsync(d.rq.in.get(), in, m * sizeof(rt_surface_point), hipMemcpyHostToDevice, d.stream));
                in = d.rq.in.get();
                res = d.rq.out.get();
            }
            HIPCHK(ctx, hipEventRecord(d.rq_events[2 * c], d.stream));
            HIPCHK(ctx, rt::launch_direct_light(sc, a, in, res, (uint32_t)m, counters, d.counters.get(), d.stream));
            HIPCHK(ctx, hipEventRecord(d.rq_events[2 * c + 1], d.stream));
            if (!pin.device) HIPCHK(ctx, hipMemcpyAsync(out + off, res, m * sizeof(rt_lighting), hipMemcpyDeviceToHost, d.stream));
        }
        return RT_OK;
    };
    for (size_t j = 0; j < nd; j++)
        if (count[j] > 0)
            if (int rc = enqueue(j)) {
                drain_streams(ctx);
                return rc;
            }
    double kernel_ms = 0.0;
    unsigned long long segments = 0, nodes = 0, tris = 0, answered = 0, entries = 0;
    for (size_t j = 0; j < nd; j++) {
        if (count[j] == 0) continue;
        DeviceState& d = ctx->devs[j];
        hipError_t e = hipSetDevice(d.device);
        if (e == hipSuccess) e = hipStreamSynchronize(d.stream);
        if (e != hipSuccess) {
            drain_streams(ctx);
            return ctx->fail(RT_ERR_HIP, "%s: device %d: %s", fn, d.device, hipGetErrorString(e));
        }
        double ms = 0.0;
        for (size_t c = 0; c * chunk < count[j]; c++) {
            float cm = 0.0f;
            HIPCHK(ctx, hipEventElapsedTime(&cm, d.rq_events[2 * c], d.rq_events[2 * c + 1]));
            ms += cm;
        }
        kernel_ms = std::max(kernel_ms, ms);
        unsigned long long cn[RT_CNT_DIAG];
        HIPCHK(ctx, hipMemcpy(cn, d.counters.get(), sizeof cn, hipMemcpyDeviceToHost));
        segments += cn[RT_CNT_SHADOW];
        nodes += cn[RT_CNT_NODE_VISITS];
        tris += cn[RT_CNT_TRI_TESTS];
        answered += cn[RT_CNT_DL_GRID_ANSWERED];
        entries += cn[RT_CNT_DL_GRID_ENTRIES];
    }
    if (counters) ctx->grid_diag[0] = answered, ctx->grid_diag[1] = entries;
    rt_stats& st = ctx->stats;
    st.rays = st.shadow_rays = segments;
    st.primary_rays = st.continuation_rays = st.pixels = 0;
    st.node_visits = counters ? nodes : 0;
    st.tri_tests = counters ? tris : 0;
    st.kernel_ms = kernel_ms;
    st.wall_ms = now_ms() - w0;
    return RT_OK;
}

int run_radiance(rt_ctx* ctx, const rt_ray* rays, size_t n, const rt_path_params* p, rt_path_result* out) {
    const char* fn = "rt_radiance";
    const double w0 = now_ms();
    if (!ctx) return RT_ERR_BAD_ARG;
    if (n == 0) return RT_OK;
    if (!rays || !p || !out) return ctx->fail(RT_ERR_BAD_ARG, "%s: %s is NULL with n = %zu", fn, !rays ? "rays" : !p ? "params" : "out", n);
    if (p->samples < 1 || p->samples > RT_PATH_MAX_SAMPLES) return ctx->fail(RT_ERR_BAD_ARG, "%s: samples %u (1 .. %u)", fn, p->samples, RT_PATH_MAX_SAMPLES);
    if (p->max_bounces > RT_MAX_BOUNCES) return ctx->fail(RT_ERR_BAD_ARG, "%s: max_bounces %u (0 .. %u)", fn, p->max_bounces, RT_MAX_BOUNCES);
    if ((uint64_t)p->first_sample + p->samples > (1ull << 32))
        return ctx->fail(RT_ERR_BAD_ARG, "%s: first_sample %u + samples %u passes 2^32", fn, p->first_sample, p->samples);
    const uint32_t known = RT_QUERY_COUNTERS | RT_PATH_NO_SHADOWS | RT_PATH_CAMERA_DRAWS;
    if (p->flags & ~known) return ctx->fail(RT_ERR_BAD_ARG, "%s: unknown flag bits 0x%x", fn, p->flags & ~known);
    if (!ctx->uploaded) return ctx->fail(RT_ERR_NOT_UPLOADED, "%s: no scene uploaded", fn);
    if (int rcp = sync_pending(ctx)) return rcp;
    QueryPtr pin, pout;
    if (int rc = classify_ptr(ctx, fn, "rays", rays, pin)) return rc;
    if (int rc = classify_ptr(ctx, fn, "out", out, pout)) return rc;
    if (pin.device != pout.device || pin.dev != pout.dev)
        return ctx->fail(RT_ERR_BAD_ARG, "%s: rays and out must both be host memory or both device memory of the same device", fn);
    const rt::PathArgs args{p->samples, p->max_bounces, p->seed, p->first_sample, (p->flags & RT_PATH_NO_SHADOWS) ? 0u : 1u,
                            (p->flags & RT_PATH_CAMERA_DRAWS) ? 1u : 0u};
    const size_t chunk = std::max<size_t>(1, RT_QUERY_CHUNK / p->samples);
    const bool counters = (p->flags & RT_QUERY_COUNTERS) != 0;
    const size_t nd = ctx->devs.size();
    std::vector<size_t> first(nd, 0), count(nd, 0);
    if (pin.device) count[pin.dev] = n;
    else
        for (size_t j = 0; j < nd; j++) first[j] = n * j / nd, count[j] = n * (j + 1) / nd - first[j];
    auto enqueue = [&](size_t j) -> int {
        DeviceState& d = ctx->devs[j];
        HIPCHK(ctx, hipSetDevice(d.device));
        const DevScene sc = scene_for(ctx, d);
        const size_t chunks = (count[j] + chunk - 1) / chunk;
        if (int rc = ensure_query_events(ctx, d, pin.device ? 2 : 2 * chunks)) return rc;
        const size_t most = std::min<size_t>(count[j], chunk);
        if (args.samples > 1) HIPCHK(ctx, d.rq.paths.reserve(most * args.samples * sizeof(uint4)));
        if (!pin.device) {
            HIPCHK(ctx, d.rq.in.reserve(most * sizeof(rt_ray)));
            HIPCHK(ctx, d.rq.out.reserve(most * sizeof(rt_path_result)));
        }
        HIPCHK(ctx, hipMemsetAsync(d.counters.get(), 0, RT_CNT_DIAG * sizeof(unsigned long long), d.stream));
        for (size_t c = 0; c < chunks; c++) {
            const size_t off = first[j] + c * chunk, m = std::min<size_t>(chunk, first[j] + count[j] - off);
            const void* in = rays + off;
            void* res = out + off;
            if (!pin.device) {
                HIPCHK(ctx, hipMemcpyAsync(d.rq.in.get(), in, m * sizeof(rt_ray), hipMemcpyHostToDevice, d.stream));
                in = d.rq.in.get();
                res = d.rq.out.get();
            }
            if (!pin.device || c == 0) HIPCHK(ctx, hipEventRecord(d.rq_events[pin.device ? 0 : 2 * c], d.stream));
            HIPCHK(ctx, rt::launch_path_query(sc, args, in, off, (uint32_t)m, d.rq.paths.get(), res, counters, d.counters.get(), d.stream));
            if (!pin.device || c + 1 == chunks) HIPCHK(ctx, hipEventRecord(d.rq_events[pin.device ? 1 : 2 * c + 1], d.stream));
            if (!pin.device) HIPCHK(ctx, hipMemcpyAsync(out + off, res, m * sizeof(rt_path_result), hipMemcpyDeviceToHost, d.stream));
        }
        return RT_OK;
    };
    for (size_t j = 0; j < nd; j++)
        if (count[j] > 0)
            if (int rc = enqueue(j)) {
                drain_streams(ctx);
                return rc;
            }
    double kernel_ms = 0.0;
    unsigned long long camera = 0, continuation = 0, shadow = 0, nodes = 0, tris = 0;
    for (size_t j = 0; j < nd; j++) {
        if (count[j] == 0) continue;
        DeviceState& d = ctx->devs[j];
        hipError_t e = hipSetDevice(d.device);
        if (e == hipSuccess) e = hipStreamSynchronize(d.stream);
        if (e != hipSuccess) {
            drain_streams(ctx);
            return ctx->fail(RT_ERR_HIP, "%s: device %d: %s", fn, d.device, hipGetErrorString(e));
// ... 404 lines not shown
```

gpu_raytracer_amd/csrc/rt_scene.cpp:

```cpp
#include "rt_internal.h"

#define RT_DEVICE_BUILD_MIN_TRIS 1024u

namespace rti {
namespace {

template <class T>
int upload_array(rt_ctx* ctx, DevBuf<T>& dst, const std::vector<T>& src) {
    dst.reset();
    if (src.empty()) return RT_OK;
    HIPCHK(ctx, dst.reserve(src.size() * sizeof(T)));
    HIPCHK(ctx, hipMemcpy(dst.get(), src.data(), src.size() * sizeof(T), hipMemcpyHostToDevice));
    return RT_OK;
}

int tree_method(size_t n_tris) {
    int method = 2;
    if (const char* e = std::getenv("RT_BUILD_METHOD")) method = std::atoi(e);
    if (method == 2 && n_tris < RT_DEVICE_BUILD_MIN_TRIS) method = 0;
    return method;
}

rt::BvhBuildOptions knob_build_options() {
    rt::BvhBuildOptions opt;
// ... 400 lines not shown
                HIPCHK(ctx, hipSetDevice(s.device));
                HIPCHK(ctx, hipMemcpy(staged.data(), s.scene.verts.get(), vbytes, hipMemcpyDeviceToHost));
                HIPCHK(ctx, hipSetDevice(d.device));
            }
            HIPCHK(ctx, hipMemcpy(d.scene.verts.get(), staged.data(), vbytes, hipMemcpyHostToDevice));
        }
    }
    drop_grids(ctx);
    if (!rebuild) {
        if (int rc = ensure_refit_view(ctx)) return rc;
        if (ctx->rf_n_dropped) {
            DeviceState& d = ctx->devs[0];
            uint32_t flag = 0;
            HIPCHK(ctx, hipSetDevice(d.device));
            HIPCHK(ctx, hipMemsetAsync(d.refit.flag.get(), 0, sizeof(uint32_t), d.stream));
            HIPCHK(ctx, rt::launch_refit_any_finite(d.refit.dropped.get(), ctx->rf_n_dropped, d.scene.verts.get(), d.refit.flag.get(), d.stream));
            HIPCHK(ctx, hipMemcpyAsync(&flag, d.refit.flag.get(), sizeof flag, hipMemcpyDeviceToHost, d.stream));
            HIPCHK(ctx, hipStreamSynchronize(d.stream));
            rebuild = flag != 0;
        }
    }
    if (rebuild) {
        std::vector<float> staged;
        const float* hv = reinterpret_cast<const float*>(vertices);
        if (pv.device) {
            if (int rc = read_positions(ctx, staged)) return rc;
            hv = staged.data();
        }
        gather_positions(ctx, hv);
        ctx->host_geometry_stale = false;
        TreeBuild tb;
        if (int rc = build_tree(ctx, ctx->build_tris, tree_method(ctx->build_tris.size()), knob_build_options(), tb)) return rc;
        if (int rc = install_tree(ctx, tb)) return rc;
        *stat_flags = RT_STAT_REBUILT;
        return RT_OK;
    }
    const std::vector<uint32_t>& lv = ctx->rf_level_first;
    for (auto& d : ctx->devs) {
        HIPCHK(ctx, hipSetDevice(d.device));
        HIPCHK(ctx, hipEventRecord(d.ev0, d.stream));
        HIPCHK(ctx, rt::launch_refit_tris(d.scene.tris.get(), d.refit.vidx.get(), d.scene.verts.get(), ctx->scene_counts.n_tris, d.stream));
        for (size_t l = lv.size() - 1; l-- > 0;)
            HIPCHK(ctx, rt::launch_refit_nodes(d.scene.nodes.get(), d.refit.boxes.get(), d.scene.tris.get(), d.refit.vidx.get(), d.scene.verts.get(), d.refit.order.get() + lv[l], lv[l + 1] - lv[l], d.stream));
        HIPCHK(ctx, hipEventRecord(d.ev1, d.stream));
    }
    for (auto& d : ctx->devs) {
        HIPCHK(ctx, hipSetDevice(d.device));
        HIPCHK(ctx, hipStreamSynchronize(d.stream));
        float ms = 0.0f;
        HIPCHK(ctx, hipEventElapsedTime(&ms, d.ev0, d.ev1));
        *kernel_ms = std::max(*kernel_ms, (double)ms);
    }
    if (pv.device) ctx->host_geometry_stale = true;
    else {
        gather_positions(ctx, reinterpret_cast<const float*>(vertices));
        ctx->host_geometry_stale = false;
    }
    *stat_flags = RT_STAT_REFIT;
    return RT_OK;
}

}

void free_scene(DeviceState& d) {
    (void)hipSetDevice(d.device);
    d.scene = {};
    d.grids = {};
    d.rq = {};
    d.refit = {};
    d.acc = {};
    d.ad = {};
}

int ensure_grids(rt_ctx* ctx, DeviceState& d) {
    if (d.grids.tried) return RT_OK;
    if (int rc = sync_host_geometry(ctx)) return rc;
    d.grids.tried = true;
    const uint32_t n_lights = (uint32_t)ctx->host_lights.size(), tree_tris = ctx->scene_counts.n_tris;
    bool grids_on = true;
    rt::ShadowGridOptions gopt;
    if (const char* e = std::getenv("RT_SHADOW_GRID")) grids_on = std::atoi(e) != 0;
    if (const char* e = std::getenv("RT_SHADOW_GRID_RES")) gopt.res_point = (uint32_t)std::atoi(e), gopt.res_dir = 2u * (uint32_t)std::atoi(e);
    if (const char* e = std::getenv("RT_SHADOW_GRID_HEAVY")) gopt.heavy = (uint32_t)std::atoi(e);
    if (const char* e = std::getenv("RT_SHADOW_GRID_MEAN")) gopt.max_mean_list = std::atof(e), gopt.max_heavy_share = 1.0;
    if (!grids_on || n_lights == 0 || n_lights > RT_WF_MAX_LIGHTS || tree_tris == 0) return RT_OK;
    const double t0 = now_ms();
    HIPCHK(ctx, hipSetDevice(d.device));
    HIPCHK(ctx, hipStreamSynchronize(d.stream));
    std::vector<DevShadowGrid> hg(n_lights);
    bool any = false;
    size_t free_b = 0, total_b = 0;
    HIPCHK(ctx, hipMemGetInfo(&free_b, &total_b));
    rt::ShadowGridOptions lopt = gopt;
    lopt.max_bytes = free_b / 4 / n_lights;
    lopt.max_entries = std::min<uint64_t>(gopt.max_entries, lopt.max_bytes / (RT_SG_ENTRY_QUADS * sizeof(uint4)));
    struct Guard {
        DeviceState& d;
        bool ok = false;
        ~Guard() { if (!ok) { d.grids = {}; d.grids.tried = true; } }
    } guard{d};
    uint64_t bytes = 0;
    bool partial = false;
    for (uint32_t i = 0; i < n_lights; i++) {
        rt::ShadowGridBuild gb;
        const hipError_t e = rt::shadow_grid_build(d.scene.tris.get(), tree_tris, ctx->host_lights[i], ctx->box_lo, ctx->box_hi, lopt, d.stream, &gb);
        if (e != hipSuccess) {
            (void)hipGetLastError();
            gb = rt::ShadowGridBuild{};
        }
        hg[i] = gb.grid;
        if (gb.blocks) d.grids.allocs.emplace_back(gb.blocks, 0);
        if (gb.overflow) d.grids.allocs.emplace_back(gb.overflow, 0);
        if (gb.grid.kind != RT_SG_KIND_NONE) bytes += gb.bytes;
        any = any || gb.grid.kind != RT_SG_KIND_NONE;
        if (gb.grid.kind == RT_SG_KIND_NONE && gb.n_entries != 0) partial = true;
        d.grids.info.push_back(gb);
    }
    if (any && partial) {
        HIPCHK(ctx, hipDeviceSynchronize());
        std::vector<rt::ShadowGridBuild> info = std::move(d.grids.info);
        d.grids = {};
        d.grids.tried = true;
        for (rt::ShadowGridBuild& g : info) g.grid = DevShadowGrid{}, g.blocks = g.overflow = nullptr, g.bytes = 0;
        d.grids.info = std::move(info);
        any = false;
        bytes = 0;
    }
    if (any) {
        if (int rc = upload_array(ctx, d.grids.table, hg)) return rc;
        HIPCHK(ctx, hipDeviceSynchronize());
    }
    if (&d == &ctx->devs[0]) {
        ctx->stats.grid_bytes = bytes;
        ctx->stats.grid_build_ms = now_ms() - t0;
    }
    guard.ok = true;
    return RT_OK;
}

}

using namespace rti;

extern "C" {

int rt_upload_scene(rt_ctx* ctx, const rt_sphere* spheres, uint32_t n_spheres, const rt_light* lights, uint32_t n_lights,
                    const rt_vertex* vertices, uint32_t n_vertices, const rt_triangle* triangles, uint32_t n_triangles,
                    const rt_material* materials, uint32_t n_materials, const rt_bvh_node* ref_nodes, uint32_t n_ref_nodes,
                    const uint32_t* ref_tri_indices, uint32_t n_ref_tri_indices) {
    if (!ctx) return RT_ERR_BAD_ARG;
    if ((n_spheres && !spheres) || (n_lights && !lights) || (n_vertices && !vertices) || (n_triangles && !triangles) ||
        (n_materials && !materials))
        return ctx->fail(RT_ERR_BAD_ARG, "rt_upload_scene: null array with non-zero count");
    if (ref_nodes) {
        for (uint32_t i = 0; i < n_ref_nodes; i++) {
            const rt_bvh_node& n = ref_nodes[i];
            bool leaf = n.left_child == RT_INVALID_INDEX;
            if (!leaf && (n.left_child >= n_ref_nodes || (n.right_child != RT_INVALID_INDEX && n.right_child >= n_ref_nodes)))
                return ctx->fail(RT_ERR_BAD_ARG, "reference BVH node %u has a child out of range", i);
            if (leaf && ref_tri_indices && (uint64_t)n.triangle_start + n.triangle_count > n_ref_tri_indices)
                return ctx->fail(RT_ERR_BAD_ARG, "reference BVH leaf %u exceeds triangle_indices", i);
        }
    }
    std::vector<rt_triangle> tris(triangles, triangles + n_triangles);
    return upload_common(ctx, spheres, n_spheres, lights, n_lights, vertices, n_vertices, tris, {}, materials, n_materials);
}

int rt_upload_scene_packed(rt_ctx* ctx, const uint32_t* md, size_t n_u32, const rt_scene_metadata_offsets* off,
                           const rt_triangle* const tri_buffers[3], const uint32_t tri_counts[3], uint32_t triangles_per_buffer,
                           const rt_material* materials, uint32_t n_materials) {
    if (!ctx) return RT_ERR_BAD_ARG;
    if (!off || (n_u32 && !md) || !tri_buffers || !tri_counts || (n_materials && !materials))
        return ctx->fail(RT_ERR_BAD_ARG, "rt_upload_scene_packed: null argument");
    auto section_ok = [&](uint32_t o, uint32_t count, uint32_t words) { return (uint64_t)o + (uint64_t)count * words <= n_u32; };
    if (!section_ok(off->spheres_offset, off->spheres_count, RT_SPHERE_WORDS) ||
        !section_ok(off->lights_offset, off->lights_count, RT_LIGHT_WORDS) ||
        !section_ok(off->bvh_nodes_offset, off->bvh_nodes_count, RT_BVH_NODE_WORDS) ||
        !section_ok(off->triangle_indices_offset, off->triangle_indices_count, 1) ||
        !section_ok(off->vertices_offset, off->vertices_count, RT_VERTEX_WORDS))
        return ctx->fail(RT_ERR_BAD_ARG, "rt_upload_scene_packed: a metadata section exceeds the buffer (%zu words)", n_u32);
    const rt_sphere* spheres = reinterpret_cast<const rt_sphere*>(md + off->spheres_offset);
    const rt_light* lights = reinterpret_cast<const rt_light*>(md + off->lights_offset);
    const rt_vertex* vertices = reinterpret_cast<const rt_vertex*>(md + off->vertices_offset);
    std::vector<rt_triangle> tris;
    std::vector<uint32_t> prim_ids;
    for (int b = 0; b < 3; b++) {
        if (tri_counts[b] == 0) continue;
        if (!tri_buffers[b]) return ctx->fail(RT_ERR_BAD_ARG, "rt_upload_scene_packed: triangle buffer %d is null", b);
        if (triangles_per_buffer == 0 || tri_counts[b] > triangles_per_buffer)
            return ctx->fail(RT_ERR_BAD_ARG, "rt_upload_scene_packed: buffer %d holds %u > triangles_per_buffer %u", b, tri_counts[b],
                             triangles_per_buffer);
        for (uint32_t i = 0; i < tri_counts[b]; i++) {
            tris.push_back(tri_buffers[b][i]);
            prim_ids.push_back((uint32_t)b * triangles_per_buffer + i);
        }
    }
    return upload_common(ctx, spheres, off->spheres_count, lights, off->lights_count, vertices, off->vertices_count, tris, prim_ids,
                         materials, n_materials);
}

int rt_upload_textures(rt_ctx* ctx, const rt_texture_info* textures, uint32_t n_textures, const uint8_t* texture_data, size_t n_bytes) {
    if (!ctx) return RT_ERR_BAD_ARG;
    if ((n_textures && !textures) || (n_bytes && !texture_data)) return ctx->fail(RT_ERR_BAD_ARG, "rt_upload_textures: null array with non-zero count");
    for (uint32_t i = 0; i < n_textures; i++)
        if ((uint64_t)textures[i].offset + textures[i].size > n_bytes)
            return ctx->fail(RT_ERR_BAD_ARG, "rt_upload_textures: texture %u (offset %u, %u bytes) exceeds the %zu bytes of texture data", i,
                             textures[i].offset, textures[i].size, n_bytes);
    ctx->n_textures = n_textures;
    ctx->texture_bytes = n_bytes;
    ctx->stats.n_textures = n_textures;
    ctx->stats.texture_bytes = n_bytes;
// ... 53 lines not shown
```

gpu_raytracer_amd/csrc/shadow_grid.h:

```cpp
#ifndef RT_SHADOW_GRID_H
#define RT_SHADOW_GRID_H

#include <hip/hip_runtime.h>

#include "device_layout.h"

struct DevShadowGrid {
    uint32_t kind;
    uint32_t res;
    uint32_t n_cells;
    uint32_t heavy;
    float origin[3];
    float scale;
    float axis_u[3];
    float u0;
    float axis_v[3];
    float v0;
    float axis_w[3];
    float key_top;
    float limit_margin;
    uint32_t near_begin, near_end;
    uint32_t _pad;
    const uint4* blocks;
    const uint4* overflow;
    uint32_t _pad2[4];
};

static_assert(sizeof(DevShadowGrid) == 128, "DevShadowGrid is staged in LDS and uploaded as an array");

#define RT_SG_EXT_EPS 0.001f
#define RT_SG_KIND_NONE 0u
#define RT_SG_KIND_CUBE 1u
#define RT_SG_KIND_ORTHO 2u
#define RT_SG_ENTRY_QUADS 3u
#define RT_SG_BLOCK_QUADS 8u
#define RT_SG_BLOCK_ENTRIES 2u
#ifndef RT_SG_SORTED_PREFIX
#define RT_SG_SORTED_PREFIX 32u
#endif

namespace rt {

struct ShadowGridOptions {
    uint32_t res_point = 1024;
    uint32_t res_dir = 2048;
    uint32_t heavy = 128;
    uint64_t max_entries = 400ull << 20;
    uint64_t max_bytes = ~0ull;
    double max_mean_list = 32.0;
    double max_heavy_share = 0.05;
};

struct ShadowGridBuild {
    DevShadowGrid grid{};
    void* blocks = nullptr;
    void* overflow = nullptr;
    uint64_t bytes = 0;
    uint64_t n_entries = 0;
    uint32_t near_count = 0;
    uint32_t longest = 0;
    uint32_t heavy_cells = 0;
    uint32_t filled_cells = 0;
};

hipError_t shadow_grid_build(const DevTri* d_tris, uint32_t n_records, const DevLight& light, const float lo[3], const float hi[3],
                             const ShadowGridOptions& opt, hipStream_t stream, ShadowGridBuild* out);

}
#endif
```

gpu_raytracer_amd/csrc/shadow_grid.hip:

```cpp
#include "shadow_grid.h"

#include <hip/hip_runtime.h>

#include <cstring>

#include <rocprim/device/device_scan.hpp>

#include <algorithm>
#include <cmath>
#include <cstdio>

namespace {

#define SG_EXT_EPS RT_SG_EXT_EPS
#define SG_MARGIN_CELLS 0.5f
#define SG_MAX_CONE_CELLS 8.0f

struct SgParams {
    const DevTri* tris;
    uint32_t n_records;
    uint32_t kind, res, n_cells;
    float L[3];
    float eps_eff;
    float scale;
// ... 203 lines not shown
            py[k] = (poly[k].y / z + 1.0f) * p.scale;
        }
        if (!ok) {
            const float qx[4] = {0.0f, (float)p.res, (float)p.res, 0.0f}, qy[4] = {0.0f, 0.0f, (float)p.res, (float)p.res};
            sg_raster<FILL>(p, face * p.res * p.res, qx, qy, 4, mc, tri, r_min, lane);
            continue;
        }
        sg_raster<FILL>(p, face * p.res * p.res, px, py, n, mc, tri, r_min, lane);
    }
}

__global__ __launch_bounds__(256) void k_sg_sum(const uint32_t* __restrict__ count, uint32_t n, uint32_t heavy, unsigned long long* out) {
    unsigned long long s = 0;
    uint32_t filled = 0, over = 0;
    for (uint32_t i = blockIdx.x * blockDim.x + threadIdx.x; i < n; i += gridDim.x * blockDim.x) {
        const uint32_t c = count[i];
        s += c;
        if (i + 1 < n) filled += c != 0u, over += c > heavy;
    }
    for (int off = 32; off > 0; off >>= 1) {
        s += __shfl_down(s, off, 64);
        filled += __shfl_down(filled, off, 64);
        over += __shfl_down(over, off, 64);
    }
    if ((threadIdx.x & 63u) == 0 && s) {
        atomicAdd(&out[0], s);
        atomicAdd(&out[1], (unsigned long long)filled);
        atomicAdd(&out[2], (unsigned long long)over);
    }
}

__global__ __launch_bounds__(256) void k_sg_overflow(const uint32_t* __restrict__ count, uint32_t* __restrict__ ovf, uint32_t n_cells) {
    const uint32_t c = blockIdx.x * blockDim.x + threadIdx.x;
    if (c > n_cells) return;
    const uint32_t n = count[c];
    ovf[c] = c < n_cells ? (n > RT_SG_BLOCK_ENTRIES ? n - RT_SG_BLOCK_ENTRIES : 0u) : n;
}
__global__ void k_sg_total(uint32_t* ovf_start, const uint32_t* ovf, uint32_t n) { ovf_start[n + 1] = ovf_start[n] + ovf[n]; }

__global__ __launch_bounds__(256) void k_sg_sort(const uint32_t* __restrict__ count, const uint32_t* __restrict__ ovf_start, uint4* __restrict__ blocks,
                                                 uint4* __restrict__ overflow, uint32_t n_cells, uint32_t heavy, uint32_t* __restrict__ stats) {
    const uint32_t c = blockIdx.x * blockDim.x + threadIdx.x;
    if (c > n_cells) return;
    const uint32_t n = count[c], os = ovf_start[c];
    const uint32_t in_block = c < n_cells ? RT_SG_BLOCK_ENTRIES : 0u;
    uint4* __restrict__ blk = blocks + (size_t)c * RT_SG_BLOCK_QUADS;
    auto at = [&](uint32_t i) -> uint4* { return i < in_block ? blk + 1u + RT_SG_ENTRY_QUADS * i : overflow + (size_t)(os + (i - in_block)) * RT_SG_ENTRY_QUADS; };
    if (n) atomicMax(&stats[0], n);
    if (n > 1 && n <= heavy && c < n_cells) {
        const uint32_t m = n < RT_SG_SORTED_PREFIX ? n : RT_SG_SORTED_PREFIX;
        for (uint32_t i = 0; i + 1 < n && i < m; i++) {
            uint32_t best = i, bk = at(i)[0].x, br = at(i)[2].z;
            for (uint32_t j = i + 1; j < n; j++) {
                const uint32_t k = at(j)[0].x;
                if (k < bk || (k == bk && at(j)[2].z < br)) best = j, bk = k, br = at(j)[2].z;
            }
            if (best != i) {
                uint4 *a = at(i), *b = at(best);
                const uint4 a0 = a[0], a1 = a[1], a2 = a[2];
                a[0] = b[0], a[1] = b[1], a[2] = b[2];
                b[0] = a0, b[1] = a1, b[2] = a2;
            }
        }
    }
    if (c < n_cells) blk[0] = make_uint4(n, os, n > RT_SG_BLOCK_ENTRIES ? at(RT_SG_BLOCK_ENTRIES)[0].x : 0x7F800000u, 0u);
}

__global__ __launch_bounds__(256) void k_sg_keep(const uint32_t* __restrict__ count, uint32_t* __restrict__ keep, uint32_t n_cells, uint32_t heavy) {
    const uint32_t c = blockIdx.x * blockDim.x + threadIdx.x;
    if (c > n_cells) return;
    const uint32_t n = count[c];
    const uint32_t looked_at = n <= heavy ? (n < RT_SG_SORTED_PREFIX ? n : RT_SG_SORTED_PREFIX) : 0u;
    keep[c] = c < n_cells ? (looked_at > RT_SG_BLOCK_ENTRIES ? looked_at - RT_SG_BLOCK_ENTRIES : 0u) : n;
}
__global__ __launch_bounds__(256) void k_sg_compact(const uint32_t* __restrict__ keep, const uint32_t* __restrict__ keep_start, const uint32_t* __restrict__ ovf_start,
                                                    const uint4* __restrict__ built, uint4* __restrict__ overflow, uint4* __restrict__ blocks, uint32_t n_cells) {
    const uint32_t c = blockIdx.x * blockDim.x + threadIdx.x;
    if (c > n_cells) return;
    const uint32_t n = keep[c], from = ovf_start[c], to = keep_start[c];
    for (uint32_t q = 0; q < n * RT_SG_ENTRY_QUADS; q++) overflow[(size_t)to * RT_SG_ENTRY_QUADS + q] = built[(size_t)from * RT_SG_ENTRY_QUADS + q];
    if (c < n_cells) reinterpret_cast<uint32_t*>(blocks + (size_t)c * RT_SG_BLOCK_QUADS)[1] = to;
}

#define SG_CHK(call)                  \
    do {                              \
        hipError_t e_ = (call);       \
        if (e_ != hipSuccess) {       \
            cleanup();                \
            return e_;                \
        }                             \
    } while (0)

uint32_t pow2_at_least(double v) {
    uint32_t r = 1;
    while ((double)r < v && r < (1u << 30)) r <<= 1;
    return r;
}

}

namespace rt {

hipError_t shadow_grid_build(const DevTri* d_tris, uint32_t n_records, const DevLight& light, const float lo[3], const float hi[3],
                             const ShadowGridOptions& opt, hipStream_t stream, ShadowGridBuild* out) {
    *out = ShadowGridBuild{};
    if (n_records == 0 || (n_records % RT_DEV_LEAF_STRIDE) != 0) return hipSuccess;
    for (int a = 0; a < 3; a++)
        if (!std::isfinite(lo[a]) || !std::isfinite(hi[a]) || !(lo[a] <= hi[a])) return hipSuccess;
    SgParams p{};
    p.tris = d_tris;
    p.n_records = n_records;
    double c_max = 0.0;
    for (int a = 0; a < 3; a++) c_max = std::max(c_max, std::max(std::fabs((double)lo[a]), std::fabs((double)hi[a])));
    const double n_real = (double)n_records / RT_DEV_LEAF_STRIDE;
    float limit_margin = 0.0f;
    if (light.light_type == 0) {
        double w[3] = {light.neg_ndir[0], light.neg_ndir[1], light.neg_ndir[2]};
        const double wl = std::sqrt(w[0] * w[0] + w[1] * w[1] + w[2] * w[2]);
        if (!std::isfinite(wl) || !(std::fabs(wl - 1.0) < 1e-3)) return hipSuccess;
        int least = 0;
        for (int a = 1; a < 3; a++)
            if (std::fabs(w[a]) < std::fabs(w[least])) least = a;
        double ax[3] = {0, 0, 0};
        ax[least] = 1.0;
        double u[3] = {w[1] * ax[2] - w[2] * ax[1], w[2] * ax[0] - w[0] * ax[2], w[0] * ax[1] - w[1] * ax[0]};
        const double ul = std::sqrt(u[0] * u[0] + u[1] * u[1] + u[2] * u[2]);
        for (int a = 0; a < 3; a++) u[a] /= ul;
        double v[3] = {w[1] * u[2] - w[2] * u[1], w[2] * u[0] - w[0] * u[2], w[0] * u[1] - w[1] * u[0]};
        double umin = 1e300, umax = -1e300, vmin = 1e300, vmax = -1e300, smax = -1e300;
        for (int k = 0; k < 8; k++) {
            const double x[3] = {(k & 1) ? hi[0] : lo[0], (k & 2) ? hi[1] : lo[1], (k & 4) ? hi[2] : lo[2]};
            const double pu = x[0] * u[0] + x[1] * u[1] + x[2] * u[2], pv = x[0] * v[0] + x[1] * v[1] + x[2] * v[2];
            const double ps = x[0] * w[0] + x[1] * w[1] + x[2] * w[2];
            umin = std::min(umin, pu), umax = std::max(umax, pu), vmin = std::min(vmin, pv), vmax = std::max(vmax, pv), smax = std::max(smax, ps);
        }
        const uint32_t res = std::min(std::max(pow2_at_least(4.0 * std::sqrt(n_real)), 32u), std::max(32u, opt.res_dir));
        const double extent = std::max(std::max(umax - umin, vmax - vmin), 1e-6) * (1.0 + 4.0 / res) + 1e-5 * c_max + 1e-30;
        const double scale = res / extent;
        const double margin = SG_MARGIN_CELLS + 1.6e-6 * c_max * scale * 4.0;
        if (!std::isfinite(scale) || !(margin < 3.0)) return hipSuccess;
        p.kind = RT_SG_KIND_ORTHO;
        p.res = res;
        p.n_cells = res * res;
        p.scale = (float)scale;
        p.u0 = (float)(0.5 * (umin + umax) - 0.5 * extent);
        p.v0 = (float)(0.5 * (vmin + vmax) - 0.5 * extent);
        p.key_top = (float)(smax + 1.0 + 1e-3 * c_max);
        p.margin_cells = (float)margin;
        for (int a = 0; a < 3; a++) p.au[a] = (float)u[a], p.av[a] = (float)v[a], p.aw[a] = light.neg_ndir[a];
        limit_margin = (float)(1.0e-4 + 4.0e-6 * c_max);
    } else {
        double d_max = 0.0;
        for (int a = 0; a < 3; a++) {
            if (!std::isfinite(light.position[a])) return hipSuccess;
            c_max = std::max(c_max, std::fabs((double)light.position[a]));
            const double far_side = std::max(std::fabs((double)light.position[a] - lo[a]), std::fabs((double)light.position[a] - hi[a]));
            d_max += far_side * far_side;
        }
        d_max = std::sqrt(d_max);
        const double eps_eff = SG_EXT_EPS * 1.01 + 2.0e-6 * (d_max + c_max);
        if (!std::isfinite(eps_eff) || !(eps_eff < 0.01 * (d_max + 1e-30) + SG_EXT_EPS * 2.0)) return hipSuccess;
        const uint32_t res = std::min(std::max(pow2_at_least(2.0 * std::sqrt(n_real)), 16u), std::max(16u, opt.res_point));
        p.kind = RT_SG_KIND_CUBE;
        p.res = res;
        p.n_cells = 6u * res * res;
        p.scale = 0.5f * (float)res;
        p.eps_eff = (float)eps_eff;
        p.margin_cells = SG_MARGIN_CELLS;
        for (int a = 0; a < 3; a++) p.L[a] = light.position[a];
        limit_margin = (float)(2.0 * eps_eff + 1.0e-5 * d_max);
    }

    uint32_t *count = nullptr, *ovf = nullptr, *ovf_start = nullptr, *keep = nullptr, *keep_start = nullptr, *stats = nullptr;
    unsigned long long* total64 = nullptr;
    uint4 *blocks = nullptr, *overflow = nullptr, *built = nullptr;
    void* temp = nullptr;
    auto cleanup = [&]() {
        (void)hipFree(count);
        (void)hipFree(ovf);
        (void)hipFree(ovf_start);
        (void)hipFree(keep);
        (void)hipFree(keep_start);
        (void)hipFree(stats);
        (void)hipFree(total64);
        (void)hipFree(blocks);
        (void)hipFree(overflow);
        (void)hipFree(built);
        (void)hipFree(temp);
    };
    const size_t lists = (size_t)p.n_cells + 1;
    SG_CHK(hipMalloc((void**)&count, lists * 4));
    SG_CHK(hipMalloc((void**)&ovf, lists * 4));
    SG_CHK(hipMalloc((void**)&ovf_start, (lists + 1) * 4));
    SG_CHK(hipMalloc((void**)&keep, lists * 4));
    SG_CHK(hipMalloc((void**)&keep_start, (lists + 1) * 4));
    SG_CHK(hipMalloc((void**)&stats, 2 * 4));
    SG_CHK(hipMalloc((void**)&total64, 3 * 8));
    SG_CHK(hipMemsetAsync(total64, 0, 3 * 8, stream));
    SG_CHK(hipMemsetAsync(count, 0, lists * 4, stream));
    SG_CHK(hipMemsetAsync(stats, 0, 2 * 4, stream));
    p.cell_count = count;
    const dim3 grid((n_records + 3u) / 4u), block(256);
    hipLaunchKernelGGL(k_sg_raster<false>, grid, block, 0, stream, p);
    SG_CHK(hipGetLastError());
    hipLaunchKernelGGL(k_sg_sum, dim3(1024), dim3(256), 0, stream, count, (uint32_t)lists, opt.heavy, total64);
    hipLaunchKernelGGL(k_sg_overflow, dim3((uint32_t)((lists + 255) / 256)), dim3(256), 0, stream, count, ovf, p.n_cells);
    size_t temp_bytes = 0;
    SG_CHK(rocprim::exclusive_scan(nullptr, temp_bytes, ovf, ovf_start, 0u, lists, rocprim::plus<uint32_t>(), stream));
    SG_CHK(hipMalloc(&temp, temp_bytes ? temp_bytes : 16));
    SG_CHK(rocprim::exclusive_scan(temp, temp_bytes, ovf, ovf_start, 0u, lists, rocprim::plus<uint32_t>(), stream));
    hipLaunchKernelGGL(k_sg_total, dim3(1), dim3(1), 0, stream, ovf_start, ovf, (uint32_t)(lists - 1));
    hipLaunchKernelGGL(k_sg_keep, dim3((uint32_t)((lists + 255) / 256)), dim3(256), 0, stream, count, keep, p.n_cells, opt.heavy);
    SG_CHK(rocprim::exclusive_scan(temp, temp_bytes, keep, keep_start, 0u, lists, rocprim::plus<uint32_t>(), stream));
    hipLaunchKernelGGL(k_sg_total, dim3(1), dim3(1), 0, stream, keep_start, keep, (uint32_t)(lists - 1));
    uint32_t tail[2] = {0, 0}, built_tail[2] = {0, 0};
    unsigned long long sums[3] = {0, 0, 0};
    SG_CHK(hipMemcpyAsync(tail, keep_start + lists - 1, 8, hipMemcpyDeviceToHost, stream));
    SG_CHK(hipMemcpyAsync(built_tail, ovf_start + lists - 1, 8, hipMemcpyDeviceToHost, stream));
    SG_CHK(hipMemcpyAsync(sums, total64, 3 * 8, hipMemcpyDeviceToHost, stream));
    SG_CHK(hipStreamSynchronize(stream));
    const unsigned long long total = sums[0];
    out->n_entries = total;
    out->filled_cells = (uint32_t)sums[1];
    out->heavy_cells = (uint32_t)sums[2];
    const uint32_t near_count = tail[1] - tail[0];
    const bool long_lists = (double)total > opt.max_mean_list * (double)std::max<uint64_t>(1, sums[1]) || (double)sums[2] > opt.max_heavy_share * (double)sums[1];
    if (total == 0 || total > std::min<uint64_t>(opt.max_entries, 0xFFFFFFFFull / RT_SG_ENTRY_QUADS) || near_count > std::min(opt.heavy, 64u) || long_lists) {
        cleanup();
        return hipSuccess;
    }
    const size_t block_bytes = (size_t)p.n_cells * RT_SG_BLOCK_QUADS * sizeof(uint4), ovf_bytes = ((size_t)tail[1] + 1) * RT_SG_ENTRY_QUADS * sizeof(uint4);
    if ((uint64_t)block_bytes + ovf_bytes > opt.max_bytes) {
        cleanup();
        return hipSuccess;
    }
    SG_CHK(hipMalloc((void**)&blocks, block_bytes));
    SG_CHK(hipMalloc((void**)&built, ((size_t)built_tail[1] + 1) * RT_SG_ENTRY_QUADS * sizeof(uint4)));
    SG_CHK(hipMemsetAsync(blocks, 0, block_bytes, stream));
    SG_CHK(hipMemsetAsync(count, 0, lists * 4, stream));
    p.ovf_start = ovf_start;
    p.blocks = blocks;
    p.overflow = built;
    hipLaunchKernelGGL(k_sg_raster<true>, grid, block, 0, stream, p);
    SG_CHK(hipGetLastError());
    hipLaunchKernelGGL(k_sg_sort, dim3((uint32_t)((lists + 255) / 256)), dim3(256), 0, stream, count, ovf_start, blocks, built, p.n_cells, opt.heavy, stats);
    SG_CHK(hipGetLastError());
    if (tail[1] == built_tail[1]) {
        overflow = built;
        built = nullptr;
    } else {
        SG_CHK(hipMalloc((void**)&overflow, ovf_bytes));
        hipLaunchKernelGGL(k_sg_compact, dim3((uint32_t)((lists + 255) / 256)), dim3(256), 0, stream, keep, keep_start, ovf_start, built, overflow, blocks, p.n_cells);
        SG_CHK(hipGetLastError());
    }
    uint32_t st[2] = {0, 0};
    SG_CHK(hipMemcpyAsync(st, stats, 8, hipMemcpyDeviceToHost, stream));
    SG_CHK(hipStreamSynchronize(stream));
    (void)hipFree(count);
    (void)hipFree(ovf);
    (void)hipFree(ovf_start);
    (void)hipFree(keep);
    (void)hipFree(keep_start);
    (void)hipFree(stats);
    (void)hipFree(total64);
    (void)hipFree(temp);
    (void)hipFree(built);

    DevShadowGrid& g = out->grid;
    g.kind = p.kind;
    g.res = p.res;
    g.n_cells = p.n_cells;
    g.heavy = opt.heavy;
    for (int a = 0; a < 3; a++) g.origin[a] = p.L[a], g.axis_u[a] = p.au[a], g.axis_v[a] = p.av[a], g.axis_w[a] = p.aw[a];
    g.scale = p.scale;
    g.u0 = p.u0;
    g.v0 = p.v0;
    g.key_top = p.key_top;
    g.limit_margin = limit_margin;
    g.near_begin = tail[0];
    g.near_end = tail[1];
    g.blocks = blocks;
    g.overflow = overflow;
    out->blocks = blocks;
    out->overflow = overflow;
    out->bytes = block_bytes + ovf_bytes;
    out->near_count = near_count;
    out->longest = st[0];
    return hipSuccess;
}

}
```

gpu_raytracer_amd/csrc/shadow_grid_walk.h:

```cpp
#ifndef RT_SHADOW_GRID_WALK_H
#define RT_SHADOW_GRID_WALK_H

#include "device_common.h"
#include "shadow_grid.h"

namespace rtdev {

#define RT_KEEP4(v) asm volatile("" : "+v"((v).x), "+v"((v).y), "+v"((v).z), "+v"((v).w))
__device__ __forceinline__ void stage_lights(DevLight* __restrict__ s_lights, const DevScene& sc) {
    const uint32_t words = sc.n_lights * (uint32_t)(sizeof(DevLight) / 4);
    const uint32_t* __restrict__ src = reinterpret_cast<const uint32_t*>(sc.lights);
    uint32_t* dst = reinterpret_cast<uint32_t*>(s_lights);
    for (uint32_t i = threadIdx.x; i < words; i += blockDim.x) dst[i] = src[i];
    __syncthreads();
}

#ifndef RT_WF_GRID_WALK
#define RT_WF_GRID_WALK 31
#endif
static_assert(EXT_EPS == RT_SG_EXT_EPS, "the light grids' dilation is derived from the shadow segments' origin offset");
static_assert(RT_WF_GRID_WALK < RT_SG_SORTED_PREFIX, "a walk may only look at the ordered part of a list");
enum : uint32_t { GRID_VISIBLE = 0u, GRID_OCCLUDED = 1u, GRID_FORWARD = 2u, GRID_PENDING = 3u };
struct GridPending {
    V3 o, d;
    float dist, limit;
    uint32_t at;
    uint32_t i, count;
};
static_assert(RT_SG_BLOCK_ENTRIES == 2u, "grid_segment_head tests the block's two entries by name");
typedef uint32_t sg_u32x4 __attribute__((ext_vector_type(4)));
__device__ __forceinline__ uint4 sg_ldg4(const uint4* p) {
    const sg_u32x4 v = *reinterpret_cast<const __attribute__((address_space(1))) sg_u32x4*>(reinterpret_cast<uintptr_t>(p));
    return make_uint4(v.x, v.y, v.z, v.w);
}
template <bool COUNT>
__device__ __forceinline__ uint32_t grid_segment_head(const DevScene& sc, const DevLight& light, const DevShadowGrid& g, V3 point, V3 normal, GridPending& pend,
                                                      uint32_t& n_tests, uint32_t& n_entries) {
    V3 d;
    float dist;
    shadow_segment(light, point, d, dist);
    const V3 o = point + normal * EXT_EPS;
    Hit hit;
    hit.t = dist;
    hit.prim = RT_PRIM_MISS;
    hit.slot = 0;
    test_spheres(sc, o, d, hit, RT_MIN_RAY_DISTANCE);
    if (hit.prim != RT_PRIM_MISS) return GRID_OCCLUDED;
    const uint32_t kind = g.kind;
    uint32_t cell = 0xFFFFFFFFu;
    float limit = 0.0f;
    if (kind == RT_SG_KIND_CUBE) {
        const float wx = -d.x, wy = -d.y, wz = -d.z;
        const float ax = fabsf(wx), ay = fabsf(wy), az = fabsf(wz);
        const uint32_t a = (ax >= ay && ax >= az) ? 0u : (ay >= az ? 1u : 2u);
        const float wa = a == 0u ? wx : (a == 1u ? wy : wz), wb_ = a == 0u ? wy : (a == 1u ? wz : wx), wc = a == 0u ? wz : (a == 1u ? wx : wy);
        const float inv = __builtin_amdgcn_rcpf(fabsf(wa));
        const float fu = (wb_ * inv + 1.0f) * g.scale, fv = (wc * inv + 1.0f) * g.scale;
        const uint32_t top = g.res - 1u;
        const uint32_t ix = min((uint32_t)max((int)floorf(fu), 0), top), iy = min((uint32_t)max((int)floorf(fv), 0), top);
        cell = ((2u * a + (wa < 0.0f ? 1u : 0u)) * g.res + iy) * g.res + ix;
        limit = dist + g.limit_margin;
    } else if (kind == RT_SG_KIND_ORTHO) {
        const float fu = (dot(o, ld3(g.axis_u)) - g.u0) * g.scale, fv = (dot(o, ld3(g.axis_v)) - g.v0) * g.scale;
        const float r = (float)g.res;
        if (fu >= 0.0f && fu < r && fv >= 0.0f && fv < r) cell = (uint32_t)fv * g.res + (uint32_t)fu;
        limit = (g.key_top - dot(o, ld3(g.axis_w))) + g.limit_margin;
    } else {
        return GRID_FORWARD;
    }
    if (cell == 0xFFFFFFFFu && g.near_begin == g.near_end) return GRID_VISIBLE;
    uint4 hd = make_uint4(0u, 0u, 0x7F800000u, 0u), q0 = hd, q1 = hd, q2 = hd;
    const uint4* __restrict__ blk = g.blocks + (size_t)(cell == 0xFFFFFFFFu ? 0u : cell) * RT_SG_BLOCK_QUADS;
    if (cell != 0xFFFFFFFFu) {
        hd = sg_ldg4(blk);
        q0 = sg_ldg4(blk + 1), q1 = sg_ldg4(blk + 2), q2 = sg_ldg4(blk + 3);
        RT_KEEP4(hd);
        RT_KEEP4(q0);
        RT_KEEP4(q1);
        RT_KEEP4(q2);
    }
    const uint32_t count = hd.x;
    if (count > g.heavy) return GRID_FORWARD;
    const uint4* __restrict__ ovf = g.overflow;
    for (uint32_t k = g.near_begin; k < g.near_end; k++) {
        const uint4 n0 = sg_ldg4(ovf + 3 * (size_t)k), n1 = sg_ldg4(ovf + 3 * (size_t)k + 1), n2 = sg_ldg4(ovf + 3 * (size_t)k + 2);
        if (COUNT) n_tests++;
        float t;
        if (moller_trumbore(v3(__uint_as_float(n0.y), __uint_as_float(n0.z), __uint_as_float(n0.w)), v3(__uint_as_float(n1.x), __uint_as_float(n1.y), __uint_as_float(n1.z)),
                            v3(__uint_as_float(n1.w), __uint_as_float(n2.x), __uint_as_float(n2.y)), o, d, t) &&
            t > RT_MIN_RAY_DISTANCE && t < dist)
            return GRID_OCCLUDED;
    }
    if (count == 0u || !(__uint_as_float(q0.x) < limit)) return GRID_VISIBLE;
    float t;
    if (COUNT) n_entries++, n_tests++;
    if (moller_trumbore(v3(__uint_as_float(q0.y), __uint_as_float(q0.z), __uint_as_float(q0.w)), v3(__uint_as_float(q1.x), __uint_as_float(q1.y), __uint_as_float(q1.z)),
                        v3(__uint_as_float(q1.w), __uint_as_float(q2.x), __uint_as_float(q2.y)), o, d, t) &&
        t > RT_MIN_RAY_DISTANCE && t < dist)
        return GRID_OCCLUDED;
    if (count == 1u) return GRID_VISIBLE;
    q0 = sg_ldg4(blk + 4), q1 = sg_ldg4(blk + 5), q2 = sg_ldg4(blk + 6);
    if (!(__uint_as_float(q0.x) < limit)) return GRID_VISIBLE;
    if (COUNT) n_entries++, n_tests++;
    if (moller_trumbore(v3(__uint_as_float(q0.y), __uint_as_float(q0.z), __uint_as_float(q0.w)), v3(__uint_as_float(q1.x), __uint_as_float(q1.y), __uint_as_float(q1.z)),
                        v3(__uint_as_float(q1.w), __uint_as_float(q2.x), __uint_as_float(q2.y)), o, d, t) &&
        t > RT_MIN_RAY_DISTANCE && t < dist)
        return GRID_OCCLUDED;
    if (count == 2u || !(__uint_as_float(hd.z) < limit)) return GRID_VISIBLE;
    pend.o = o, pend.d = d, pend.dist = dist, pend.limit = limit;
    pend.at = hd.y, pend.i = 2u, pend.count = count;
    return GRID_PENDING;
}
template <bool COUNT>
__device__ __forceinline__ uint32_t grid_walk_on(const DevShadowGrid& g, GridPending& pend, uint32_t trips, uint32_t& n_tests, uint32_t& n_entries) {
    const uint4* __restrict__ ovf = g.overflow;
    for (uint32_t k = 0; k < trips; k++) {
// ... 23 lines not shown
```

gpu_raytracer_amd/csrc/wavefront.h:

```cpp
#ifndef RT_WAVEFRONT_H
#define RT_WAVEFRONT_H

#include <hip/hip_runtime.h>

#include "../../include/rt_hip.h"
#include "device_layout.h"
#include "shadow_grid.h"

namespace rt {

enum WfCounter : uint32_t {
    WF_EXT_COUNT = 0,
    WF_EXT_NEXT = 1,
    WF_SHADOW2_COUNT = 2,
    WF_SHADOW_COUNT = 3,
    WF_EXT_CURSOR = 4,
    WF_SHADOW_CURSOR = 5,
    WF_EXT_WINDOW = 6,
    WF_SHADOW_WINDOW = 7,
    WF_EXT_WINDOW_NEXT = 8,
    WF_SHADOW2_CURSOR = 9,
    WF_SHADOW2_WINDOW = 10,
    WF_UNUSED_11 = 11,
    WF_FB_COUNT = 12,
    WF_FB_CURSOR = 13,
    WF_N_COUNTERS = 16
};

enum WfTotal : uint32_t {
    WF_TOTAL_CAMERA = 0,
    WF_TOTAL_CONTINUATION = 1,
    WF_TOTAL_SHADOW = 2,
    WF_TOTAL_NODE_VISITS = 3,
    WF_TOTAL_TRI_TESTS = 4,
    WF_TOTAL_STACK_MAX = 5,
    WF_TOTAL_EMPTY_VISITS = 6,
    WF_TOTAL_CHILDREN_ENTERED = 7,
    WF_TOTAL_NODE_STEPS = 8,
    WF_TOTAL_LEAF_STEPS = 9,
    WF_TOTAL_LEAF_LANES = 10,
    WF_TOTAL_LEAF_TRIPS = 11,
    WF_TOTAL_REFILLS = 12,
    WF_TOTAL_GRID_ANSWERED = 13,
    WF_TOTAL_GRID_ENTRIES = 14,
    WF_TOTAL_ERROR = 15,
    WF_N_TOTALS = 16
};

struct WfBuffers {
    float4* ray_o;
    float4* ray_d;
    uint4* hit;
    float4* thr;
    float4* rad;
    float4* next_o;
    float4* next_d;
    float4* next_thr;
    float4* next_rad;
    float4* vtx;
    float4* sample_rad;
    uint32_t* pxy;
    uint32_t* q_ext[2];
    uint32_t* q_shadow;
    uint32_t* q_shadow2;
    const DevShadowGrid* grids;
    uint32_t* counters;
    unsigned long long* totals;
    float4* accum;
    uint32_t q_ext_cap;
    uint32_t q_shadow_cap;
    uint32_t state_cap;
    uint32_t* stack_ovf;
    uint32_t ovf_entries;
    uint32_t n_blocks;
    uint32_t batch;
    uint32_t capacity;
    uint32_t* beam_count;
    uint32_t* beam_ref;
    float* beam_dist;
    uint32_t probe;
};

#ifndef RT_BEAM_CAP
#define RT_BEAM_CAP 128u
#endif
#define RT_BEAM_OVERFLOW 0x80000000u
#ifndef RT_WF8_LDS_STACK
#define RT_WF8_LDS_STACK 8
#endif
#define RT_WF_MAX_LIGHTS 32u
#define RT_WF_ID_MASK 0x07FFFFFFu

uint32_t wf_shading_blocks();
size_t wf_state_slots(size_t paths);
size_t wf_state_slots_for(size_t paths, size_t producing_waves);
size_t wf_queue_slots(size_t max_entries, uint32_t per_lane);
size_t wf_queue_slots_for(size_t max_entries, uint32_t per_lane, size_t producing_waves);
uint32_t wf_pick_window(uint32_t iterations, uint32_t per_lane);
uint32_t wf_persistent_waves();
hipError_t wf_beams(const DevScene& sc, const DevFrame& fr, const WfBuffers& wb, hipStream_t s);
hipError_t wf_generate(const DevScene& sc, const DevFrame& fr, const WfBuffers& wb, const DevTargets& tg, uint32_t first_sample, uint32_t n_samples, hipStream_t s);
inline bool wf_runs_shadow_grid(const DevFrame& fr, const WfBuffers& wb) { return !(fr.flags & RT_FLAG_NO_SHADOWS) && wb.grids; }
hipError_t wf_bounce(const DevScene& sc, const DevFrame& fr, const WfBuffers& wb, uint32_t iteration, uint32_t n_samples, bool counters, hipStream_t s,
                     hipEvent_t* grid_events = nullptr);
hipError_t wf_resolve(const DevFrame& fr, const WfBuffers& wb, const DevTargets& tg, uint32_t n_samples, uint32_t first_sample, bool first_batch, bool last_batch,
                      hipStream_t s);

}
#endif
```

gpu_raytracer_amd/csrc/wavefront.hip:

```cpp
#include "wavefront.h"
#include <cstdlib>

#include <algorithm>

#include "device_common.h"
#include "shadow_grid_walk.h"

using namespace rtdev;

#ifndef RT_WF_REFILL
#define RT_WF_REFILL 16
#endif
#ifndef RT_WF_CHUNK
#define RT_WF_CHUNK 256
#endif
#ifndef RT_WF_ADAPTIVE_CHUNK
#define RT_WF_ADAPTIVE_CHUNK 1
#endif
#ifndef RT_WF_WINDOW
#define RT_WF_WINDOW 512
#endif
#ifndef RT_WF_BLOCK_MAJOR
#define RT_WF_BLOCK_MAJOR 1
#endif
// ... 700 lines not shown
        }
        n_park += (uint32_t)__popcll(pm);
    };
    auto walk_parked = [&]() {
        const uint32_t take = min(n_park, 64u), first = n_park - take;
        const bool have = lane < take;
        GridPending pd = {};
        uint32_t entry = 0, outcome = GRID_VISIBLE;
        if (have) {
            const uint32_t s = first + lane;
            pd.o = v3(__uint_as_float(park[0][s]), __uint_as_float(park[1][s]), __uint_as_float(park[2][s]));
            pd.d = v3(__uint_as_float(park[3][s]), __uint_as_float(park[4][s]), __uint_as_float(park[5][s]));
            pd.dist = __uint_as_float(park[6][s]), pd.limit = __uint_as_float(park[7][s]);
            pd.at = park[8][s];
            const uint32_t ic = park[9][s];
            pd.i = ic & 0xFFu, pd.count = ic >> 8;
            entry = park[10][s];
            outcome = grid_walk_on<COUNT>(s_grids[entry >> 27], pd, RT_WF_GRID_PASS, n_tests, n_entries);
            if (outcome == GRID_OCCLUDED) atomicAnd(reinterpret_cast<uint32_t*>(&wb.vtx[2 * (size_t)(entry & RT_WF_ID_MASK) + 1]) + 3, ~(1u << (entry >> 27)));
            if (COUNT && outcome <= GRID_OCCLUDED) n_answered++;
        }
        n_park = first;
        park_push(have && outcome == GRID_PENDING, pd, entry);
        hand_on(have && outcome == GRID_FORWARD, entry, false);
    };
    const uint32_t count = wb.counters[rt::WF_EXT_COUNT];
    const uint32_t stride = gridDim.x * blockDim.x;
    uint32_t id_next = blockIdx.x * blockDim.x + threadIdx.x < count ? queue[blockIdx.x * blockDim.x + threadIdx.x] : WF_SENTINEL;
    for (uint32_t base = blockIdx.x * blockDim.x; base < count; base += stride) {
        const uint32_t id = id_next;
        const uint32_t i_next = base + stride + threadIdx.x;
        id_next = i_next < count ? queue[i_next] : WF_SENTINEL;
        uint32_t want = 0;
        V3 point = v3(0, 0, 0), normal = point;
        if (id != WF_SENTINEL) {
            float4 vp = wb.vtx[2 * (size_t)id], vn = wb.vtx[2 * (size_t)id + 1];
            RT_KEEP4(vp);
            RT_KEEP4(vn);
            point = f4v(vp), normal = f4v(vn);
            if (__float_as_uint(vp.w) != 0xFFFFFFFFu) want = __float_as_uint(vn.w);
        }
        uint32_t occluded = 0;
        for (uint32_t li = 0; li < sc.n_lights; li++) {
            const bool mine = (want >> li) & 1u;
            if (__ballot(mine) == 0ull) continue;
            uint32_t outcome = GRID_VISIBLE;
            GridPending pd = {};
            if (mine) {
                outcome = grid_segment_head<COUNT>(sc, s_lights[li], s_grids[li], point, normal, pd, n_tests, n_entries);
                if (outcome == GRID_OCCLUDED) occluded |= 1u << li;
                if (COUNT && outcome <= GRID_OCCLUDED) n_answered++;
            }
            const uint32_t entry = id | (li << 27);
            park_push(mine && outcome == GRID_PENDING, pd, entry);
            hand_on(mine && outcome == GRID_FORWARD, entry, false);
            while (n_park >= 64u) walk_parked();
        }
        if (occluded != 0u) atomicAnd(reinterpret_cast<uint32_t*>(&wb.vtx[2 * (size_t)id + 1]) + 3, ~occluded);
    }
    while (n_park != 0u) walk_parked();
    hand_on(false, 0u, true);
    if (COUNT) {
        const unsigned long long t = wave_sum(n_tests), a = wave_sum(n_answered), en = wave_sum(n_entries);
        if ((threadIdx.x & 63u) == 0) {
            atomicAdd(&wb.totals[rt::WF_TOTAL_TRI_TESTS], t);
            atomicAdd(&wb.totals[rt::WF_TOTAL_GRID_ANSWERED], a);
            atomicAdd(&wb.totals[rt::WF_TOTAL_GRID_ENTRIES], en);
        }
    }
}

__device__ __forceinline__ void wf_end_path(const rt::WfBuffers& wb, uint32_t origin, V3 radiance) {
    wb.sample_rad[origin] = make_float4(radiance.x, radiance.y, radiance.z, 0.0f);
}
__device__ __forceinline__ uint32_t wf_origin(const rt::WfBuffers& wb, uint32_t id) { return __float_as_uint(wb.ray_d[id].w); }

__global__ __launch_bounds__(256, RT_WF_SHADE_WAVES) void k_wf_shade(DevScene sc, DevFrame fr, rt::WfBuffers wb, const uint32_t* __restrict__ queue) {
    __shared__ DevLight s_lights[RT_WF_MAX_LIGHTS];
    if (wb.totals[rt::WF_TOTAL_ERROR] != 0ull) return;
    stage_lights(s_lights, sc);
    const uint32_t count = wb.counters[rt::WF_EXT_COUNT];
    const bool shadows = (fr.flags & RT_FLAG_NO_SHADOWS) == 0;
    const bool to_grids = shadows && wb.grids != nullptr;
    const uint32_t stride = gridDim.x * blockDim.x;
    OutWindow win = {0u, 0u};
    uint32_t n_shadow = 0;
    const uint32_t window = pick_window((count + stride - 1u) / stride, max(1u, sc.n_lights));
    if (blockIdx.x == 0 && threadIdx.x == 0) wb.counters[rt::WF_SHADOW_WINDOW] = window;
    uint32_t id_next = blockIdx.x * blockDim.x + threadIdx.x < count ? queue[blockIdx.x * blockDim.x + threadIdx.x] : WF_SENTINEL;
    for (uint32_t base = blockIdx.x * blockDim.x; base < count; base += stride) {
        const uint32_t id = id_next;
        const uint32_t i_next = base + stride + threadIdx.x;
        id_next = i_next < count ? queue[i_next] : WF_SENTINEL;
        const bool have = id != WF_SENTINEL;
        bool vertex = false;
        V3 point = v3(0, 0, 0), normal = point;
        uint32_t material_id = 0;
        DevMaterial m = {};
        if (have) {
            uint4 h = wb.hit[id];
            asm volatile("" : "+v"(h.x), "+v"(h.y), "+v"(h.z), "+v"(h.w));
            if (h.w == RT_PRIM_MISS) {
                const V3 radiance = f4v(wb.rad[id]) + RT_SKY() * f4v(wb.thr[id]);
                wf_end_path(wb, wf_origin(wb, id), radiance);
            } else {
                point = v3(__uint_as_float(h.x), __uint_as_float(h.y), __uint_as_float(h.z));
                surface_at(sc, (h.w & RT_PRIM_SPHERE_FLAG) != 0, h.w & ~RT_PRIM_SPHERE_FLAG, point, normal, material_id);
                if (material_id >= sc.n_materials) {
                    const V3 radiance = f4v(wb.rad[id]) + RT_MAGENTA() * f4v(wb.thr[id]);
                    wf_end_path(wb, wf_origin(wb, id), radiance);
                } else {
                    vertex = true;
                    m = load_material(sc, material_id);
                    wb.vtx[2 * (size_t)id] = make_float4(point.x, point.y, point.z, __uint_as_float(material_id));
                    if (!shadows) wb.vtx[2 * (size_t)id + 1] = make_float4(normal.x, normal.y, normal.z, 0.0f);
                }
            }
        }
        if (have && !vertex) wb.vtx[2 * (size_t)id] = make_float4(0.0f, 0.0f, 0.0f, __uint_as_float(0xFFFFFFFFu));
        if (shadows) {
            uint32_t mask = 0;
            if (vertex) {
                for (uint32_t li = 0; li < sc.n_lights; li++) {
                    V3 sdir;
                    float sdist;
                    const V3 contrib = light_contribution(s_lights[li], m, point, normal, sdir, sdist);
                    if (needs_shadow_segment(contrib)) mask |= 1u << li;
                }
            }
            if (vertex) wb.vtx[2 * (size_t)id + 1] = make_float4(normal.x, normal.y, normal.z, __uint_as_float(mask));
            if (to_grids) {
                n_shadow += (uint32_t)__popc(mask);
                continue;
            }
#if RT_WF_SHADOW_LIGHT_MAJOR
            uint32_t total = 0;
            for (uint32_t li = 0; li < sc.n_lights; li++) total += (uint32_t)__popcll(__ballot((mask >> li) & 1u));
            if (total) {
                uint32_t at = window_reserve(wb.q_shadow, &wb.counters[rt::WF_SHADOW_COUNT], win, window, 0u, 0u, total, wb.q_shadow_cap, &wb.totals[rt::WF_TOTAL_ERROR]);
                n_shadow += (uint32_t)__popc(mask);
                const unsigned long long below = (1ull << (threadIdx.x & 63u)) - 1ull;
                for (uint32_t li = 0; at != WF_NO_SLOT && li < sc.n_lights; li++) {
                    const bool want = (mask >> li) & 1u;
                    const unsigned long long b = __ballot(want);
                    if (want) wb.q_shadow[at + (uint32_t)__popcll(b & below)] = id | (li << 27);
                    at += (uint32_t)__popcll(b);
                }
            }
#else
            const uint32_t mine = (uint32_t)__popc(mask);
            const uint32_t incl = wave_incl_scan(mine), total = __shfl(incl, WAVE - 1, WAVE);
            if (total) {
                uint32_t at = window_reserve(wb.q_shadow, &wb.counters[rt::WF_SHADOW_COUNT], win, window, mine, incl, total, wb.q_shadow_cap, &wb.totals[rt::WF_TOTAL_ERROR]);
                n_shadow += mine;
                while (mask && at != WF_NO_SLOT) {
                    const uint32_t li = (uint32_t)__ffs((int)mask) - 1u;
                    mask &= mask - 1u;
                    wb.q_shadow[at++] = id | (li << 27);
                }
            }
#endif
        }
    }
    window_close(wb.q_shadow, win);
    const unsigned long long ns = wave_sum(n_shadow);
    if ((threadIdx.x & 63u) == 0 && ns) atomicAdd(&wb.totals[rt::WF_TOTAL_SHADOW], ns);
}

__global__ void k_wf_advance(rt::WfBuffers wb) {
    if (threadIdx.x != 0 || blockIdx.x != 0) return;
    uint32_t* c = wb.counters;
    c[rt::WF_EXT_COUNT] = c[rt::WF_EXT_NEXT];
    c[rt::WF_EXT_WINDOW] = c[rt::WF_EXT_WINDOW_NEXT];
    c[rt::WF_EXT_NEXT] = 0;
    c[rt::WF_SHADOW_COUNT] = 0;
    c[rt::WF_SHADOW2_COUNT] = 0;
    c[rt::WF_SHADOW2_CURSOR] = 0;
    c[rt::WF_EXT_CURSOR] = 0;
    c[rt::WF_SHADOW_CURSOR] = 0;
}

__global__ __launch_bounds__(256, RT_WF_SHADE_WAVES) void k_wf_finish(DevScene sc, DevFrame fr, rt::WfBuffers wb, const uint32_t* __restrict__ queue,
                                                  uint32_t* __restrict__ next_queue) {
    __shared__ DevLight s_lights[RT_WF_MAX_LIGHTS];
    if (wb.totals[rt::WF_TOTAL_ERROR] != 0ull) return;
    stage_lights(s_lights, sc);
    const uint32_t count = wb.counters[rt::WF_EXT_COUNT];
    const bool shadows = (fr.flags & RT_FLAG_NO_SHADOWS) == 0;
    const uint32_t stride = gridDim.x * blockDim.x;
    OutWindow win = {0u, 0u};
    uint32_t n_cont = 0;
    const uint32_t window = pick_window((count + stride - 1u) / stride, 1u);
    if (blockIdx.x == 0 && threadIdx.x == 0) wb.counters[rt::WF_EXT_WINDOW_NEXT] = window;
    uint32_t id_next = blockIdx.x * blockDim.x + threadIdx.x < count ? queue[blockIdx.x * blockDim.x + threadIdx.x] : WF_SENTINEL;
    for (uint32_t base = blockIdx.x * blockDim.x; base < count; base += stride) {
        bool cont = false;
        V3 norigin = v3(0.0f, 0.0f, 0.0f), ndir = norigin, throughput = norigin, radiance = norigin;
        uint32_t next_tw = 0, rng_seed = 0, ndir_origin = 0;
        const uint32_t id = id_next;
        const uint32_t i_next = base + stride + threadIdx.x;
        id_next = i_next < count ? queue[i_next] : WF_SENTINEL;
        float4 vp = make_float4(0.0f, 0.0f, 0.0f, __uint_as_float(0xFFFFFFFFu));
        float4 vn = vp, th = vp, ra = vp, rdin = vp;
        if (id != WF_SENTINEL) {
            vp = wb.vtx[2 * (size_t)id];
            vn = wb.vtx[2 * (size_t)id + 1];
            th = wb.thr[id];
            ra = wb.rad[id];
            rdin = wb.ray_d[id];
            RT_KEEP4(vp);
            RT_KEEP4(vn);
            RT_KEEP4(th);
            RT_KEEP4(ra);
            RT_KEEP4(rdin);
        }
        const uint32_t vis = __float_as_uint(vn.w);
        if (__float_as_uint(vp.w) != 0xFFFFFFFFu) {
            const V3 point = f4v(vp), normal = f4v(vn);
            const uint32_t material_id = __float_as_uint(vp.w);
            const uint32_t origin = __float_as_uint(rdin.w);
            const DevMaterial m = load_material(sc, material_id);
            throughput = f4v(th), radiance = f4v(ra);
            const uint32_t tw = __float_as_uint(th.w);
            uint32_t channel = tw & 0xFFu;
            const uint32_t depth = tw >> 8;
            SimpleRng rng = {__float_as_uint(ra.w)};
            const bool terminal = depth >= fr.max_bounce;
            const V3 lighting = ext_light_sum(s_lights, sc.n_lights, m, point, normal, terminal, shadows, [&](uint32_t li, V3, float) { return ((vis >> li) & 1u) != 0u; });
            const float tf = ext_leave_vertex(m, lighting, terminal, throughput, radiance);
            if (terminal || !ext_scatter(m, point, normal, f4v(rdin), tf, depth, rng, channel, throughput, norigin, ndir)) {
                wf_end_path(wb, origin, radiance);
            } else {
                cont = true;
                next_tw = channel | ((depth + 1u) << 8);
                rng_seed = rng.seed;
                ndir_origin = origin;
            }
        }
        const uint32_t mine = cont ? 1u : 0u;
        const uint32_t incl = wave_incl_scan(mine), total = __shfl(incl, WAVE - 1, WAVE);
        if (total) {
            const uint32_t at = window_reserve(next_queue, &wb.counters[rt::WF_EXT_NEXT], win, window, mine, incl, total, wb.state_cap, &wb.totals[rt::WF_TOTAL_ERROR]);
            if (cont && at != WF_NO_SLOT) {
                wb.next_o[at] = make_float4(norigin.x, norigin.y, norigin.z, 0.0f);
                wb.next_d[at] = make_float4(ndir.x, ndir.y, ndir.z, __uint_as_float(ndir_origin));
                wb.next_thr[at] = make_float4(throughput.x, throughput.y, throughput.z, __uint_as_float(next_tw));
                wb.next_rad[at] = make_float4(radiance.x, radiance.y, radiance.z, __uint_as_float(rng_seed));
                next_queue[at] = at;
            }
// ... 184 lines not shown
```

include/rt_hip.h:

```cpp
#ifndef RT_HIP_H
#define RT_HIP_H

#include "rt_shared.h"

#ifdef __cplusplus
extern "C" {
#endif

#define RT_OK 0
#define RT_ERR_BAD_ARG (-1)
#define RT_ERR_OOM (-2)
#define RT_ERR_HIP (-3)
#define RT_ERR_NOT_UPLOADED (-4)
#define RT_ERR_INTERNAL (-5)

#define RT_MODE_LEGACY 0u
#define RT_MODE_WAVEFRONT 1u
#define RT_MODE_EXTENDED 2u

#define RT_FLAG_COUNTERS 1u
#define RT_FLAG_NO_SHADOWS 2u
#define RT_FLAG_KERNEL_V1 4u
#define RT_FLAG_KERNEL_SM 8u
#define RT_FLAG_NO_SHADOW_GRID 16u
// ... 127 lines not shown
    float tmax;
} rt_ray;

typedef struct rt_hit {
    float t;
    float u, v;
    uint32_t prim_id;
} rt_hit;

RT_STATIC_ASSERT(sizeof(rt_ray) == 32, "rt_ray is 32 B");
RT_STATIC_ASSERT(offsetof(rt_ray, tmin) == 12 && offsetof(rt_ray, direction) == 16 && offsetof(rt_ray, tmax) == 28, "rt_ray offsets");
RT_STATIC_ASSERT(sizeof(rt_hit) == 16, "rt_hit is 16 B");
RT_STATIC_ASSERT(offsetof(rt_hit, u) == 4 && offsetof(rt_hit, v) == 8 && offsetof(rt_hit, prim_id) == 12, "rt_hit offsets");

#define RT_QUERY_COUNTERS 1u

#define RT_QUERY_CHUNK 4194304u

int rt_intersect(rt_ctx* ctx, const rt_ray* rays, size_t n, rt_hit* hits, uint32_t flags);

int rt_occluded(rt_ctx* ctx, const rt_ray* rays, size_t n, uint8_t* occluded, uint32_t flags);

#define RT_QUERY_COUNT_ALL 2u
#define RT_MULTI_HIT_MAX 16u

int rt_intersect_all(rt_ctx* ctx, const rt_ray* rays, size_t n, uint32_t max_hits,
                     rt_hit* hits,
                     uint32_t* counts,
                     uint32_t flags);

int rt_camera_rays(rt_ctx* ctx, const rt_camera* camera, uint32_t width, uint32_t height, uint32_t mode, rt_ray* out);

typedef struct rt_surface_point {
    float position[3];
    uint32_t prim_id;
    float normal[3];
    uint32_t material_id;
} rt_surface_point;

RT_STATIC_ASSERT(sizeof(rt_surface_point) == 32, "rt_surface_point is 32 B");
RT_STATIC_ASSERT(offsetof(rt_surface_point, prim_id) == 12 && offsetof(rt_surface_point, normal) == 16 && offsetof(rt_surface_point, material_id) == 28,
                 "rt_surface_point offsets");

#define RT_AO_MAX_SAMPLES 4096u

typedef struct rt_ao_params {
    uint32_t samples;
    uint32_t seed;
    float max_distance;
    float bias;
    uint32_t flags;
    uint32_t _pad[3];
} rt_ao_params;

RT_STATIC_ASSERT(sizeof(rt_ao_params) == 32, "rt_ao_params is 32 B");
RT_STATIC_ASSERT(offsetof(rt_ao_params, seed) == 4 && offsetof(rt_ao_params, max_distance) == 8 && offsetof(rt_ao_params, bias) == 12 &&
                     offsetof(rt_ao_params, flags) == 16,
                 "rt_ao_params offsets");

int rt_surface(rt_ctx* ctx, const rt_ray* rays, size_t n, rt_surface_point* out, uint32_t flags);

int rt_ambient_occlusion(rt_ctx* ctx, const rt_surface_point* points, size_t n, const rt_ao_params* params,
                         float* visibility,
                         uint32_t* unoccluded);

typedef struct rt_lighting {
    float radiance[3];
    uint32_t lit_mask;
} rt_lighting;

typedef struct rt_direct_light_params {
    float bias;
    uint32_t flags;
    uint32_t _pad[2];
} rt_direct_light_params;

RT_STATIC_ASSERT(sizeof(rt_lighting) == 16 && offsetof(rt_lighting, lit_mask) == 12, "rt_lighting is 16 B, lit_mask at 12");
RT_STATIC_ASSERT(sizeof(rt_direct_light_params) == 16 && offsetof(rt_direct_light_params, flags) == 4 && offsetof(rt_direct_light_params, _pad) == 8,
                 "rt_direct_light_params is 16 B, flags at 4");

#define RT_DIRECT_AMBIENT 4u
#define RT_DIRECT_NO_SHADOWS 8u
#define RT_DIRECT_NO_SHADOW_GRID 16u
#define RT_DIRECT_MAX_LIGHTS 32u

int rt_direct_light(rt_ctx* ctx, const rt_surface_point* points, size_t n, const rt_direct_light_params* params, rt_lighting* out);

typedef struct rt_path_params {
    uint32_t samples;
    uint32_t max_bounces;
    uint32_t seed;
    uint32_t first_sample;
    uint32_t flags;
    uint32_t _pad[3];
} rt_path_params;

typedef struct rt_path_result {
    float radiance[3];
    uint32_t segments;
} rt_path_result;

RT_STATIC_ASSERT(sizeof(rt_path_params) == 32, "rt_path_params is 32 B");
RT_STATIC_ASSERT(offsetof(rt_path_params, max_bounces) == 4 && offsetof(rt_path_params, seed) == 8 && offsetof(rt_path_params, first_sample) == 12 &&
                     offsetof(rt_path_params, flags) == 16 && offsetof(rt_path_params, _pad) == 20,
                 "rt_path_params offsets");
RT_STATIC_ASSERT(sizeof(rt_path_result) == 16 && offsetof(rt_path_result, segments) == 12, "rt_path_result is 16 B, segments at 12");

#define RT_PATH_NO_SHADOWS 32u
#define RT_PATH_CAMERA_DRAWS 64u
#define RT_PATH_MAX_SAMPLES 4096u

int rt_radiance(rt_ctx* ctx, const rt_ray* rays, size_t n, const rt_path_params* params, rt_path_result* out);

typedef struct rt_point_query {
    float position[3];
    float radius;
} rt_point_query;

typedef struct rt_nearest {
    float position[3];
    float distance;
    float u, v;
    uint32_t prim_id;
    uint32_t material_id;
} rt_nearest;

RT_STATIC_ASSERT(sizeof(rt_point_query) == 16 && offsetof(rt_point_query, radius) == 12, "rt_point_query is 16 B, radius at 12");
RT_STATIC_ASSERT(sizeof(rt_nearest) == 32, "rt_nearest is 32 B");
RT_STATIC_ASSERT(offsetof(rt_nearest, distance) == 12 && offsetof(rt_nearest, u) == 16 && offsetof(rt_nearest, v) == 20 &&
                     offsetof(rt_nearest, prim_id) == 24 && offsetof(rt_nearest, material_id) == 28,
                 "rt_nearest offsets");

int rt_closest_point(rt_ctx* ctx, const rt_point_query* points, size_t n, rt_nearest* out, uint32_t flags);

#define RT_UPDATE_REBUILD 1u

int rt_update_geometry(rt_ctx* ctx,
                       const rt_vertex* vertices, uint32_t n_vertices,
                       const rt_sphere* spheres, uint32_t n_spheres,
                       uint32_t flags);

typedef struct rt_aov {
    float albedo[3];
    float depth;
    float normal[3];
    float coverage;
} rt_aov;

RT_STATIC_ASSERT(sizeof(rt_aov) == 32, "rt_aov is 32 B");
RT_STATIC_ASSERT(offsetof(rt_aov, depth) == 12 && offsetof(rt_aov, normal) == 16 && offsetof(rt_aov, coverage) == 28, "rt_aov offsets");

#define RT_AOV_SAMPLES_PER_LAUNCH 64u

#define RT_DENOISE_DEMODULATE 1u
#define RT_DENOISE_MAX_ITERATIONS 10u

#define RT_DENOISE_DEFAULT_ITERATIONS 2u
#define RT_DENOISE_DEFAULT_SIGMA_COLOR 4.0f
#define RT_DENOISE_DEFAULT_SIGMA_NORMAL 1.0f
#define RT_DENOISE_DEFAULT_SIGMA_DEPTH 0.1f
#define RT_DENOISE_DEFAULT_SIGMA_ALBEDO 0.3f

typedef struct rt_denoise_params {
    uint32_t width, height;
    uint32_t iterations;
    uint32_t flags;
    float sigma_color, sigma_normal, sigma_depth, sigma_albedo;
} rt_denoise_params;

// ... 22 lines not shown
```

Before: 3310.

## Add conservative shadow depth maps to resolve occluded shadow segments early

At scene preparation, a per-light depth map (default resolution 512) is built by rasterizing triangles along the light axis, alongside the existing shadow grids. During wavefront shading, each hit vertex looks up the maps for up to four lights. Segments the map reports as certainly occluded are removed from the shadow mask, so they never reach the shadow queue or grid walk. The cost is a new build kernel, extra memory, extra global loads and LDS staging in the shade kernel, and correctness that depends on the conservative margins.

```diff
diff --git a/gpu_raytracer_amd/api.py b/gpu_raytracer_amd/api.py
--- a/gpu_raytracer_amd/api.py
+++ b/gpu_raytracer_amd/api.py
@@ -31,6 +31,7 @@
 MULTI_HIT_MAX = 16
 AO_MAX_SAMPLES = 4096
 DIRECT_AMBIENT, DIRECT_NO_SHADOWS, DIRECT_NO_SHADOW_GRID = 4, 8, 16
+DIRECT_SHADOW_MAP = 128
 DIRECT_MAX_LIGHTS = 32
 PATH_NO_SHADOWS, PATH_CAMERA_DRAWS = 32, 64
 PATH_MAX_SAMPLES = 4096
@@ -56,6 +57,7 @@
     "rt_accumulated_samples",
     "rt_aovs", "rt_sample_rays", "rt_denoise",
     "rt_render_adaptive", "rt_read_adaptive",
+    "rt_debug_shadow_map",
 ]
 
 
@@ -459,6 +461,11 @@
         names = ("lights_with_grid", "entries", "bytes", "segments_answered", "entries_read") if light is None else ("kind", "res", "entries", "near", "longest", "heavy_cells", "filled_cells")
         return dict(zip(names, [int(v) for v in out]))
 
+    def debug_shadow_map(self):
+        out = (C.c_ulonglong * 8)()
+        self._check(self.lib.rt_debug_shadow_map(self._h, out))
+        return dict(zip(("lights_with_map", "bytes", "side", "keyed_cells", "segments_answered"), [int(v) for v in out]))
+
     def debug_check_bvh(self):
         out = (C.c_uint32 * 8)()
         fails = self.lib.rt_debug_check_bvh(self._h, out)
@@ -558,7 +565,7 @@
         self._check(self.lib.rt_ambient_occlusion(self._h, _addr(points), C.c_size_t(n), _p(ap), _addr(out), _addr(counts)))
         return out, counts
 
-    def direct_light(self, points, bias=1e-3, ambient=False, shadows=True, use_grids=True, out=None, counters=False):
+    def direct_light(self, points, bias=1e-3, ambient=False, shadows=True, use_grids=True, out=None, counters=False, use_map=False):
         n = _check_batch(points, "points", 8, "float32")
         try:
             bias = float(bias)
@@ -576,7 +583,7 @@
         dp = np.zeros((), dtype=T.DIRECT_LIGHT_PARAMS)
         dp["bias"] = bias
         dp["flags"] = ((DIRECT_AMBIENT if ambient else 0) | (0 if shadows else DIRECT_NO_SHADOWS) | (0 if use_grids else DIRECT_NO_SHADOW_GRID)
-                       | (QUERY_COUNTERS if counters else 0))
+                       | (QUERY_COUNTERS if counters else 0) | (DIRECT_SHADOW_MAP if use_map else 0))
         _sync_torch(points, out)
         self._check(self.lib.rt_direct_light(self._h, _addr(points), C.c_size_t(n), _p(dp), _addr(out)))
         return out
diff --git a/gpu_raytracer_amd/csrc/direct_light.h b/gpu_raytracer_amd/csrc/direct_light.h
--- a/gpu_raytracer_amd/csrc/direct_light.h
+++ b/gpu_raytracer_amd/csrc/direct_light.h
@@ -11,6 +11,7 @@
 struct DirectLightArgs {
     float bias;
     uint32_t ambient, shadows;
+    uint32_t use_map;
     const DevShadowGrid* grids;
     float lo[3], hi[3];
 };
@@ -23,6 +24,7 @@
 
 #define RT_CNT_DL_GRID_ANSWERED 6u
 #define RT_CNT_DL_GRID_ENTRIES 7u
+#define RT_CNT_DL_MAP_ANSWERED 8u
 hipError_t launch_direct_light(const DevScene& sc, const DirectLightArgs& a, const void* points, void* out, uint32_t n, bool count,
                                unsigned long long* counters, hipStream_t stream);
 
diff --git a/gpu_raytracer_amd/csrc/direct_light.hip b/gpu_raytracer_amd/csrc/direct_light.hip
--- a/gpu_raytracer_amd/csrc/direct_light.hip
+++ b/gpu_raytracer_amd/csrc/direct_light.hip
@@ -51,7 +51,7 @@
                           P.y <= a.hi[1] && P.z >= a.lo[2] && P.z <= a.hi[2];
     const V3 o = P + N * a.bias;
     uint32_t nonzero = 0, occ = 0, walk = 0;
-    uint32_t n_tests = 0, n_entries = 0, n_answered = 0;
+    uint32_t n_tests = 0, n_entries = 0, n_answered = 0, n_map = 0;
     Counts cnt = {0u, 0u};
     for (uint32_t li = 0; li < sc.n_lights; li++) {
         V3 sdir = v3(0.0f, 0.0f, 0.0f);
@@ -67,7 +67,13 @@
         if (__ballot(mine) == 0ull) continue;
         if (mine && segment_valid(o, sdir, sdist)) {
             GridPending pd = {};
-            uint32_t outcome = grid_segment_head<COUNT>(sc, s_lights[li], s_grids[li], P, N, pd, n_tests, n_entries);
+            uint32_t outcome;
+            if (a.use_map && grid_map_occluded(s_grids[li], P + N * EXT_EPS)) {
+                outcome = GRID_OCCLUDED;
+                if (COUNT) n_map++;
+            } else {
+                outcome = grid_segment_head<COUNT>(sc, s_lights[li], s_grids[li], P, N, pd, n_tests, n_entries);
+            }
             if (outcome == GRID_PENDING) outcome = grid_walk_on<COUNT>(s_grids[li], pd, RT_WF_GRID_WALK, n_tests, n_entries);
             if (COUNT && outcome <= GRID_OCCLUDED) n_answered++;
             if (outcome == GRID_OCCLUDED) occ |= 1u << li;
@@ -118,12 +124,14 @@
     const unsigned long long segments = wave_sum(shadows ? (uint32_t)__popc(nonzero) : 0u);
     if (lane == 0 && segments) atomicAdd(&counters[RT_CNT_SHADOW], segments);
     if (COUNT) {
-        const unsigned long long n0 = wave_sum(cnt.nodes), n1 = wave_sum(cnt.tris + n_tests), ga = wave_sum(n_answered), ge = wave_sum(n_entries);
+        const unsigned long long n0 = wave_sum(cnt.nodes), n1 = wave_sum(cnt.tris + n_tests), ga = wave_sum(n_answered), ge = wave_sum(n_entries),
+                                 gm = wave_sum(n_map);
         if (lane == 0) {
             atomicAdd(&counters[RT_CNT_NODE_VISITS], n0);
             atomicAdd(&counters[RT_CNT_TRI_TESTS], n1);
             atomicAdd(&counters[RT_CNT_DL_GRID_ANSWERED], ga);
             atomicAdd(&counters[RT_CNT_DL_GRID_ENTRIES], ge);
+            if (gm) atomicAdd(&counters[RT_CNT_DL_MAP_ANSWERED], gm);
         }
     }
 }
diff --git a/gpu_raytracer_amd/csrc/rt_context.cpp b/gpu_raytracer_amd/csrc/rt_context.cpp
--- a/gpu_raytracer_amd/csrc/rt_context.cpp
+++ b/gpu_raytracer_amd/csrc/rt_context.cpp
@@ -186,6 +186,20 @@
     return RT_OK;
 }
 
+int rt_debug_shadow_map(rt_ctx* ctx, unsigned long long out[8]) {
+    if (!ctx || !out) return RT_ERR_BAD_ARG;
+    for (int k = 0; k < 8; k++) out[k] = 0;
+    if (ctx->devs.empty()) return RT_OK;
+    for (const rt::ShadowGridBuild& g : ctx->devs[0].grids.info) {
+        if (g.grid.map_side == 0u) continue;
+        if (out[0]++ == 0) out[2] = g.grid.map_side;
+        out[1] += g.map_bytes;
+        out[3] += g.map_keyed;
+    }
+    out[4] = ctx->grid_diag[2];
+    return RT_OK;
+}
+
 int rt_get_stats(rt_ctx* ctx, rt_stats* out) {
     if (!ctx) return RT_ERR_BAD_ARG;
     if (!out) return ctx->fail(RT_ERR_BAD_ARG, "rt_get_stats: null out");
diff --git a/gpu_raytracer_amd/csrc/rt_frame.cpp b/gpu_raytracer_amd/csrc/rt_frame.cpp
--- a/gpu_raytracer_amd/csrc/rt_frame.cpp
+++ b/gpu_raytracer_amd/csrc/rt_frame.cpp
@@ -341,6 +341,7 @@
         HIPCHK(ctx, hipMemsetAsync(d.pipe.wf2.totals, 0, rt::WF_N_TOTALS * sizeof(unsigned long long), d.stream2));
     }
     d.pipe.wf.grids = d.pipe.wf2.grids = (f.flags & RT_FLAG_NO_SHADOW_GRID) ? nullptr : d.grids.table.get();
+    d.pipe.wf.map_lights = d.pipe.wf2.map_lights = d.pipe.wf.grids ? d.grids.map_lights : 0u;
     const char* pe = std::getenv("RT_WF_PROBE");
     d.pipe.wf.probe = d.pipe.wf2.probe = pe ? (uint32_t)std::atoi(pe) : 0u;
     d.used_two_lanes = two;
@@ -425,6 +426,7 @@
     unsigned long long segments = 0, camera = 0, continuation = 0, shadow = 0, node_visits = 0, tri_tests = 0;
     unsigned long long diag[RT_CNT_N_DIAG] = {0};
     unsigned long long grid_answered = 0, grid_entries = 0;
+    unsigned long long map_answered = 0;
 };
 
 void add_counters(FrameTotals& t, const unsigned long long (&c)[RT_CNT_SLOTS]) {
@@ -447,6 +449,7 @@
     t.diag[0] = std::max(t.diag[0], w[rt::WF_TOTAL_STACK_MAX]);
     for (int k = 1; k < RT_CNT_N_DIAG; k++) t.diag[k] += w[rt::WF_TOTAL_STACK_MAX + k];
     t.grid_answered += w[rt::WF_TOTAL_GRID_ANSWERED], t.grid_entries += w[rt::WF_TOTAL_GRID_ENTRIES];
+    t.map_answered += w[rt::WF_TOTAL_MAP_ANSWERED];
     return RT_OK;
 }
 
@@ -505,6 +508,7 @@
     st.tri_tests = counters ? t.tri_tests : 0;
     for (int k = 0; k < RT_CNT_N_DIAG; k++) ctx->diag[k] = counters ? t.diag[k] : 0;
     ctx->grid_diag[0] = counters ? t.grid_answered : 0, ctx->grid_diag[1] = counters ? t.grid_entries : 0;
+    ctx->grid_diag[2] = counters ? t.map_answered : 0;
     st.kernel_ms = t.kernel_ms, st.wall_ms = now_ms() - w0, st.flags = stat_flags;
 }
 
diff --git a/gpu_raytracer_amd/csrc/rt_internal.h b/gpu_raytracer_amd/csrc/rt_internal.h
--- a/gpu_raytracer_amd/csrc/rt_internal.h
+++ b/gpu_raytracer_amd/csrc/rt_internal.h
@@ -99,6 +99,7 @@
     struct Grids {
         DevBuf<DevShadowGrid> table;
         std::vector<DevMem> allocs;
+        uint32_t map_lights = 0;
         std::vector<rt::ShadowGridBuild> info;
         bool tried = false;
     } grids;
@@ -166,7 +167,7 @@
     uint32_t frame_w = 0, frame_h = 0, frame_tile = RT_TILE_SIZE, frame_tiles_x = 0, frame_tiles_y = 0;
     bool frame_valid = false;
     unsigned long long diag[RT_CNT_N_DIAG] = {0};
-    unsigned long long grid_diag[2] = {0};
+    unsigned long long grid_diag[3] = {0};
     double stage_ms[2] = {0.0, 0.0};
     int fail_upload_at = -1;
     uint32_t n_input_tris = 0;
diff --git a/gpu_raytracer_amd/csrc/rt_query.cpp b/gpu_raytracer_amd/csrc/rt_query.cpp
--- a/gpu_raytracer_amd/csrc/rt_query.cpp
+++ b/gpu_raytracer_amd/csrc/rt_query.cpp
@@ -283,7 +283,7 @@
     if (!ctx) return RT_ERR_BAD_ARG;
     if (n == 0) return RT_OK;
     if (!points || !p || !out) return ctx->fail(RT_ERR_BAD_ARG, "%s: %s is NULL with n = %zu", fn, !points ? "points" : !p ? "params" : "out", n);
-    const uint32_t known = RT_QUERY_COUNTERS | RT_DIRECT_AMBIENT | RT_DIRECT_NO_SHADOWS | RT_DIRECT_NO_SHADOW_GRID;
+    const uint32_t known = RT_QUERY_COUNTERS | RT_DIRECT_AMBIENT | RT_DIRECT_NO_SHADOWS | RT_DIRECT_NO_SHADOW_GRID | RT_DIRECT_SHADOW_MAP;
     if (p->flags & ~known) return ctx->fail(RT_ERR_BAD_ARG, "%s: unknown flag bits 0x%x", fn, p->flags & ~known);
     if (!std::isfinite(p->bias) || p->bias < 0.0f) return ctx->fail(RT_ERR_BAD_ARG, "%s: bias %g (finite and >= 0)", fn, (double)p->bias);
     if (!ctx->uploaded) return ctx->fail(RT_ERR_NOT_UPLOADED, "%s: no scene uploaded", fn);
@@ -299,6 +299,7 @@
     args.bias = p->bias;
     args.ambient = (p->flags & RT_DIRECT_AMBIENT) ? 1u : 0u;
     args.shadows = (p->flags & RT_DIRECT_NO_SHADOWS) ? 0u : 1u;
+    args.use_map = (p->flags & RT_DIRECT_SHADOW_MAP) ? 1u : 0u;
     const float grid_bias = RT_SG_EXT_EPS;
     const bool grids_allowed = args.shadows && !(p->flags & RT_DIRECT_NO_SHADOW_GRID) && std::memcmp(&p->bias, &grid_bias, sizeof(float)) == 0;
     rt::direct_light_box(ctx->box_lo, ctx->box_hi, args.lo, args.hi);
@@ -322,7 +323,7 @@
             HIPCHK(ctx, d.rq.in.reserve(most * sizeof(rt_surface_point)));
             HIPCHK(ctx, d.rq.out.reserve(most * sizeof(rt_lighting)));
         }
-        HIPCHK(ctx, hipMemsetAsync(d.counters.get(), 0, RT_CNT_DIAG * sizeof(unsigned long long), d.stream));
+        HIPCHK(ctx, hipMemsetAsync(d.counters.get(), 0, (RT_CNT_DL_MAP_ANSWERED + 1u) * sizeof(unsigned long long), d.stream));
         for (size_t c = 0; c < chunks; c++) {
             const size_t off = first[j] + c * chunk, m = std::min<size_t>(chunk, first[j] + count[j] - off);
             const void* in = points + off;
@@ -346,7 +347,7 @@
                 return rc;
             }
     double kernel_ms = 0.0;
-    unsigned long long segments = 0, nodes = 0, tris = 0, answered = 0, entries = 0;
+    unsigned long long segments = 0, nodes = 0, tris = 0, answered = 0, entries = 0, by_map = 0;
     for (size_t j = 0; j < nd; j++) {
         if (count[j] == 0) continue;
         DeviceState& d = ctx->devs[j];
@@ -363,15 +364,16 @@
             ms += cm;
         }
         kernel_ms = std::max(kernel_ms, ms);
-        unsigned long long cn[RT_CNT_DIAG];
+        unsigned long long cn[RT_CNT_DL_MAP_ANSWERED + 1u];
         HIPCHK(ctx, hipMemcpy(cn, d.counters.get(), sizeof cn, hipMemcpyDeviceToHost));
         segments += cn[RT_CNT_SHADOW];
         nodes += cn[RT_CNT_NODE_VISITS];
         tris += cn[RT_CNT_TRI_TESTS];
         answered += cn[RT_CNT_DL_GRID_ANSWERED];
         entries += cn[RT_CNT_DL_GRID_ENTRIES];
-    }
-    if (counters) ctx->grid_diag[0] = answered, ctx->grid_diag[1] = entries;
+        by_map += cn[RT_CNT_DL_MAP_ANSWERED];
+    }
+    if (counters) ctx->grid_diag[0] = answered, ctx->grid_diag[1] = entries, ctx->grid_diag[2] = by_map;
     rt_stats& st = ctx->stats;
     st.rays = st.shadow_rays = segments;
     st.primary_rays = st.continuation_rays = st.pixels = 0;
diff --git a/gpu_raytracer_amd/csrc/rt_scene.cpp b/gpu_raytracer_amd/csrc/rt_scene.cpp
--- a/gpu_raytracer_amd/csrc/rt_scene.cpp
+++ b/gpu_raytracer_amd/csrc/rt_scene.cpp
@@ -506,6 +506,7 @@
     if (const char* e = std::getenv("RT_SHADOW_GRID")) grids_on = std::atoi(e) != 0;
     if (const char* e = std::getenv("RT_SHADOW_GRID_RES")) gopt.res_point = (uint32_t)std::atoi(e), gopt.res_dir = 2u * (uint32_t)std::atoi(e);
     if (const char* e = std::getenv("RT_SHADOW_GRID_HEAVY")) gopt.heavy = (uint32_t)std::atoi(e);
+    if (const char* e = std::getenv("RT_SHADOW_MAP_RES")) gopt.map_res = (uint32_t)std::max(0, std::atoi(e));
     if (const char* e = std::getenv("RT_SHADOW_GRID_MEAN")) gopt.max_mean_list = std::atof(e), gopt.max_heavy_share = 1.0;
     if (!grids_on || n_lights == 0 || n_lights > RT_WF_MAX_LIGHTS || tree_tris == 0) return RT_OK;
     const double t0 = now_ms();
@@ -535,6 +536,7 @@
         hg[i] = gb.grid;
         if (gb.blocks) d.grids.allocs.emplace_back(gb.blocks, 0);
         if (gb.overflow) d.grids.allocs.emplace_back(gb.overflow, 0);
+        if (gb.map) d.grids.allocs.emplace_back(gb.map, 0);
         if (gb.grid.kind != RT_SG_KIND_NONE) bytes += gb.bytes;
         any = any || gb.grid.kind != RT_SG_KIND_NONE;
         if (gb.grid.kind == RT_SG_KIND_NONE && gb.n_entries != 0) partial = true;
@@ -545,12 +547,14 @@
         std::vector<rt::ShadowGridBuild> info = std::move(d.grids.info);
         d.grids = {};
         d.grids.tried = true;
-        for (rt::ShadowGridBuild& g : info) g.grid = DevShadowGrid{}, g.blocks = g.overflow = nullptr, g.bytes = 0;
+        for (rt::ShadowGridBuild& g : info) g.grid = DevShadowGrid{}, g.blocks = g.overflow = g.map = nullptr, g.bytes = g.map_bytes = 0, g.map_keyed = 0;
         d.grids.info = std::move(info);
         any = false;
         bytes = 0;
     }
     if (any) {
+        for (uint32_t i = 0, n = 0; i < n_lights && n < RT_WF_MAP_LIGHTS; i++)
+            if (hg[i].map_side != 0u) d.grids.map_lights |= 1u << i, n++;
         if (int rc = upload_array(ctx, d.grids.table, hg)) return rc;
         HIPCHK(ctx, hipDeviceSynchronize());
     }
diff --git a/gpu_raytracer_amd/csrc/shadow_grid.h b/gpu_raytracer_amd/csrc/shadow_grid.h
--- a/gpu_raytracer_amd/csrc/shadow_grid.h
+++ b/gpu_raytracer_amd/csrc/shadow_grid.h
@@ -20,10 +20,12 @@
     float key_top;
     float limit_margin;
     uint32_t near_begin, near_end;
-    uint32_t _pad;
+    float map_margin;
     const uint4* blocks;
     const uint4* overflow;
-    uint32_t _pad2[4];
+    const float* map;
+    uint32_t map_side;
+    float map_scale;
 };
 
 static_assert(sizeof(DevShadowGrid) == 128, "DevShadowGrid is staged in LDS and uploaded as an array");
@@ -49,13 +51,17 @@
     uint64_t max_bytes = ~0ull;
     double max_mean_list = 32.0;
     double max_heavy_share = 0.05;
+    uint32_t map_res = 512;
 };
 
 struct ShadowGridBuild {
     DevShadowGrid grid{};
     void* blocks = nullptr;
     void* overflow = nullptr;
+    void* map = nullptr;
     uint64_t bytes = 0;
+    uint64_t map_bytes = 0;
+    uint32_t map_keyed = 0;
     uint64_t n_entries = 0;
     uint32_t near_count = 0;
     uint32_t longest = 0;
diff --git a/gpu_raytracer_amd/csrc/shadow_grid.hip b/gpu_raytracer_amd/csrc/shadow_grid.hip
--- a/gpu_raytracer_amd/csrc/shadow_grid.hip
+++ b/gpu_raytracer_amd/csrc/shadow_grid.hip
@@ -309,6 +309,81 @@
     if (c < n_cells) reinterpret_cast<uint32_t*>(blocks + (size_t)c * RT_SG_BLOCK_QUADS)[1] = to;
 }
 
+#define SG_MAP_A_FACTOR 4.0f
+#define SG_F32_HALF_ULP 5.9604645e-8f
+struct SgMapParams {
+    const DevTri* tris;
+    uint32_t n_records;
+    uint32_t side;
+    float scale;
+    float au[3], av[3], aw[3];
+    float u0, v0, key_top;
+    float dilate;
+    float reach;
+    uint32_t* map;
+};
+__device__ __forceinline__ F3 cross3(F3 a, F3 b) { return f3(a.y * b.z - a.z * b.y, a.z * b.x - a.x * b.z, a.x * b.y - a.y * b.x); }
+
+__global__ __launch_bounds__(256) void k_sg_map(SgMapParams p) {
+    const uint32_t r = (uint32_t)((blockIdx.x * (size_t)blockDim.x + threadIdx.x) >> 6), lane = threadIdx.x & 63u;
+    if (r >= p.n_records) return;
+    const uint32_t leaf = r & ~(RT_DEV_LEAF_STRIDE - 1u);
+    if (r - leaf >= p.tris[leaf].leaf_count) return;
+    const DevTri t = p.tris[r];
+    const F3 v0 = f3(t.v0[0], t.v0[1], t.v0[2]), e1 = f3(t.e1[0], t.e1[1], t.e1[2]), e2 = f3(t.e2[0], t.e2[1], t.e2[2]);
+    const F3 v1 = v0 + e1, v2 = v0 + e2;
+    const float sum = (v0.x + v0.y + v0.z) + (v1.x + v1.y + v1.z) + (v2.x + v2.y + v2.z);
+    if (!(fabsf(sum) < 3.0e38f)) return;
+    const F3 au = f3(p.au[0], p.au[1], p.au[2]), av = f3(p.av[0], p.av[1], p.av[2]), d = f3(p.aw[0], p.aw[1], p.aw[2]);
+    const F3 h = cross3(d, e2);
+    const float a = dot3(e1, h);
+    if (!(fabsf(a) >= SG_MAP_A_FACTOR * 1.0e-5f)) return;
+    const float f = 1.0f / a;
+    const float l1 = sqrtf(dot3(e1, e1)), l2 = sqrtf(dot3(e2, e2));
+    const float beta = 128.0f * SG_F32_HALF_ULP * p.reach * (l1 + l2) / fabsf(a) + 1.0e-6f;
+    if (!(beta < 0.25f)) return;
+    const float pad = 64.0f * SG_F32_HALF_ULP * p.reach * l1 * l2 / fabsf(a);
+    const F3 v[3] = {v0, v1, v2};
+    float minx = 3.0e38f, maxx = -3.0e38f, miny = 3.0e38f, maxy = -3.0e38f;
+    for (int k = 0; k < 3; k++) {
+        const float x = (dot3(v[k], au) - p.u0) * p.scale, y = (dot3(v[k], av) - p.v0) * p.scale;
+        minx = fminf(minx, x), maxx = fmaxf(maxx, x), miny = fminf(miny, y), maxy = fmaxf(maxy, y);
+    }
+    const float R = (float)p.side;
+    if (!(minx < R) || !(maxx >= 0.0f) || !(miny < R) || !(maxy >= 0.0f)) return;
+    const int x0 = (int)fmaxf(floorf(minx), 0.0f), x1 = (int)fminf(floorf(maxx), R - 1.0f);
+    const int y0 = (int)fmaxf(floorf(miny), 0.0f), y1 = (int)fminf(floorf(maxy), R - 1.0f);
+    if (x1 < x0 || y1 < y0) return;
+    const uint32_t w = (uint32_t)(x1 - x0 + 1), cells = w * (uint32_t)(y1 - y0 + 1);
+    const float inv_scale = 1.0f / p.scale;
+    for (uint32_t c = lane; c < cells; c += 64u) {
+        const uint32_t row = c / w;
+        const int x = x0 + (int)(c - row * w), y = y0 + (int)row;
+        bool inside = true;
+        float kmax = -3.0e38f;
+        for (int k = 0; k < 4; k++) {
+            const float cx = (k & 1) ? (float)(x + 1) + p.dilate : (float)x - p.dilate, cy = (k & 2) ? (float)(y + 1) + p.dilate : (float)y - p.dilate;
+            const F3 X = au * (p.u0 + cx * inv_scale) + av * (p.v0 + cy * inv_scale);
+            const F3 s = X - v0;
+            const float bu = f * dot3(s, h);
+            const F3 q = cross3(s, e1);
+            const float bv = f * dot3(d, q), bt = f * dot3(e2, q);
+            inside = inside && bu >= beta && bv >= beta && 1.0f - bu - bv >= beta;
+            kmax = fmaxf(kmax, p.key_top - (dot3(X, d) + bt));
+        }
+        if (!inside) continue;
+        const float K = kmax + pad;
+        if (!(K > 0.0f) || !(K < 3.0e38f)) continue;
+        atomicMin(&p.map[(uint32_t)y * p.side + (uint32_t)x], __float_as_uint(K) + 1u);
+    }
+}
+__global__ __launch_bounds__(256) void k_sg_map_count(const uint32_t* __restrict__ map, uint32_t n, uint32_t* __restrict__ out) {
+    uint32_t keyed = 0;
+    for (uint32_t i = blockIdx.x * blockDim.x + threadIdx.x; i < n; i += gridDim.x * blockDim.x) keyed += map[i] != 0x7F800000u;
+    for (int off = 32; off > 0; off >>= 1) keyed += __shfl_down(keyed, off, 64);
+    if ((threadIdx.x & 63u) == 0 && keyed) atomicAdd(out, keyed);
+}
+
 #define SG_CHK(call)                  \
     do {                              \
         hipError_t e_ = (call);       \
@@ -341,6 +416,7 @@
     for (int a = 0; a < 3; a++) c_max = std::max(c_max, std::max(std::fabs((double)lo[a]), std::fabs((double)hi[a])));
     const double n_real = (double)n_records / RT_DEV_LEAF_STRIDE;
     float limit_margin = 0.0f;
+    double ortho_extent = 0.0;
     if (light.light_type == 0) {
         double w[3] = {light.neg_ndir[0], light.neg_ndir[1], light.neg_ndir[2]};
         const double wl = std::sqrt(w[0] * w[0] + w[1] * w[1] + w[2] * w[2]);
@@ -364,6 +440,7 @@
         const uint32_t res = std::min(std::max(pow2_at_least(4.0 * std::sqrt(n_real)), 32u), std::max(32u, opt.res_dir));
         const double extent = std::max(std::max(umax - umin, vmax - vmin), 1e-6) * (1.0 + 4.0 / res) + 1e-5 * c_max + 1e-30;
         const double scale = res / extent;
+        ortho_extent = extent;
         const double margin = SG_MARGIN_CELLS + 1.6e-6 * c_max * scale * 4.0;
         if (!std::isfinite(scale) || !(margin < 3.0)) return hipSuccess;
         p.kind = RT_SG_KIND_ORTHO;
@@ -513,6 +590,53 @@
     out->bytes = block_bytes + ovf_bytes;
     out->near_count = near_count;
     out->longest = st[0];
+
+    if (p.kind == RT_SG_KIND_ORTHO && opt.map_res != 0u) {
+        const uint32_t side = std::min(opt.map_res, p.res);
+        const double map_scale = side / ortho_extent;
+        const double dilate = 0.01 + 8.0e-6 * c_max * map_scale;
+        double diag = 0.0;
+        for (int a = 0; a < 3; a++) diag += ((double)hi[a] - lo[a]) * ((double)hi[a] - lo[a]);
+        diag = std::sqrt(diag);
+        const size_t map_bytes = (size_t)side * side * sizeof(float);
+        uint32_t *map = nullptr, *keyed = nullptr;
+        if (dilate < 0.25 && std::isfinite(map_scale) && hipMalloc((void**)&map, map_bytes) == hipSuccess && hipMalloc((void**)&keyed, 4) == hipSuccess) {
+            SgMapParams mp{};
+            mp.tris = d_tris;
+            mp.n_records = n_records;
+            mp.side = side;
+            mp.scale = (float)map_scale;
+            for (int a = 0; a < 3; a++) mp.au[a] = p.au[a], mp.av[a] = p.av[a], mp.aw[a] = p.aw[a];
+            mp.u0 = p.u0, mp.v0 = p.v0, mp.key_top = p.key_top;
+            mp.dilate = (float)dilate;
+            mp.reach = (float)(4.0 * diag + 0.01);
+            mp.map = map;
+            uint32_t n_keyed = 0;
+            hipError_t e = hipMemsetD32Async((hipDeviceptr_t)map, 0x7F800000, (size_t)side * side, stream);
+            if (e == hipSuccess) e = hipMemsetAsync(keyed, 0, 4, stream);
+            if (e == hipSuccess) {
+                hipLaunchKernelGGL(k_sg_map, grid, block, 0, stream, mp);
+                hipLaunchKernelGGL(k_sg_map_count, dim3(256), dim3(256), 0, stream, map, side * side, keyed);
+                e = hipGetLastError();
+            }
+            if (e == hipSuccess) e = hipMemcpyAsync(&n_keyed, keyed, 4, hipMemcpyDeviceToHost, stream);
+            if (e == hipSuccess) e = hipStreamSynchronize(stream);
+            if (e == hipSuccess && n_keyed != 0u) {
+                g.map = reinterpret_cast<const float*>(map);
+                g.map_side = side;
+                g.map_scale = mp.scale;
+                g.map_margin = (float)(4.0e-5 + 8.0e-6 * c_max);
+                out->map = map;
+                out->map_bytes = map_bytes;
+                out->map_keyed = n_keyed;
+                out->bytes += map_bytes;
+                map = nullptr;
+            }
+        }
+        (void)hipFree(map);
+        (void)hipFree(keyed);
+        (void)hipGetLastError();
+    }
     return hipSuccess;
 }
 
diff --git a/gpu_raytracer_amd/csrc/shadow_grid_walk.h b/gpu_raytracer_amd/csrc/shadow_grid_walk.h
--- a/gpu_raytracer_amd/csrc/shadow_grid_walk.h
+++ b/gpu_raytracer_amd/csrc/shadow_grid_walk.h
@@ -32,6 +32,22 @@
 __device__ __forceinline__ uint4 sg_ldg4(const uint4* p) {
     const sg_u32x4 v = *reinterpret_cast<const __attribute__((address_space(1))) sg_u32x4*>(reinterpret_cast<uintptr_t>(p));
     return make_uint4(v.x, v.y, v.z, v.w);
+}
+__device__ __forceinline__ float sg_ldg1(const float* p) {
+    return *reinterpret_cast<const __attribute__((address_space(1))) float*>(reinterpret_cast<uintptr_t>(p));
+}
+__device__ __forceinline__ float grid_map_fetch(const DevShadowGrid& g, V3 o, float& key) {
+    const float fu = (dot(o, ld3(g.axis_u)) - g.u0) * g.map_scale, fv = (dot(o, ld3(g.axis_v)) - g.v0) * g.map_scale;
+    const float r = (float)g.map_side;
+    key = (g.key_top - dot(o, ld3(g.axis_w))) - g.map_margin;
+    float K = __uint_as_float(0x7F800000u);
+    if (fu >= 0.0f && fu < r && fv >= 0.0f && fv < r) K = sg_ldg1(g.map + ((uint32_t)fv * g.map_side + (uint32_t)fu));
+    return K;
+}
+__device__ __forceinline__ bool grid_map_occluded(const DevShadowGrid& g, V3 o) {
+    float key;
+    const float K = grid_map_fetch(g, o, key);
+    return key > K;
 }
 template <bool COUNT>
 __device__ __forceinline__ uint32_t grid_segment_head(const DevScene& sc, const DevLight& light, const DevShadowGrid& g, V3 point, V3 normal, GridPending& pend,
diff --git a/gpu_raytracer_amd/csrc/wavefront.h b/gpu_raytracer_amd/csrc/wavefront.h
--- a/gpu_raytracer_amd/csrc/wavefront.h
+++ b/gpu_raytracer_amd/csrc/wavefront.h
@@ -44,7 +44,8 @@
     WF_TOTAL_GRID_ANSWERED = 13,
     WF_TOTAL_GRID_ENTRIES = 14,
     WF_TOTAL_ERROR = 15,
-    WF_N_TOTALS = 16
+    WF_TOTAL_MAP_ANSWERED = 16,
+    WF_N_TOTALS = 17
 };
 
 struct WfBuffers {
@@ -64,6 +65,7 @@
     uint32_t* q_shadow;
     uint32_t* q_shadow2;
     const DevShadowGrid* grids;
+    uint32_t map_lights;
     uint32_t* counters;
     unsigned long long* totals;
     float4* accum;
@@ -90,6 +92,7 @@
 #endif
 #define RT_WF_MAX_LIGHTS 32u
 #define RT_WF_ID_MASK 0x07FFFFFFu
+#define RT_WF_MAP_LIGHTS 4u
 
 uint32_t wf_shading_blocks();
 size_t wf_state_slots(size_t paths);
diff --git a/gpu_raytracer_amd/csrc/wavefront.hip b/gpu_raytracer_amd/csrc/wavefront.hip
--- a/gpu_raytracer_amd/csrc/wavefront.hip
+++ b/gpu_raytracer_amd/csrc/wavefront.hip
@@ -806,9 +806,22 @@
     const uint32_t count = wb.counters[rt::WF_EXT_COUNT];
     const bool shadows = (fr.flags & RT_FLAG_NO_SHADOWS) == 0;
     const bool to_grids = shadows && wb.grids != nullptr;
+    __shared__ DevShadowGrid s_mgrids[RT_WF_MAP_LIGHTS];
+    const uint32_t map_lights = to_grids ? wb.map_lights : 0u;
+    if (map_lights) {
+        const uint32_t gw = (uint32_t)(sizeof(DevShadowGrid) / 4), words = (uint32_t)__popc(map_lights) * gw;
+        const uint32_t* __restrict__ src = reinterpret_cast<const uint32_t*>(wb.grids);
+        uint32_t* dst = reinterpret_cast<uint32_t*>(s_mgrids);
+        for (uint32_t i = threadIdx.x; i < words; i += blockDim.x) {
+            uint32_t rest = map_lights;
+            for (uint32_t k = i / gw; k; k--) rest &= rest - 1u;
+            dst[i] = src[((uint32_t)__ffs((int)rest) - 1u) * gw + i % gw];
+        }
+        __syncthreads();
+    }
     const uint32_t stride = gridDim.x * blockDim.x;
     OutWindow win = {0u, 0u};
-    uint32_t n_shadow = 0;
+    uint32_t n_shadow = 0, n_map = 0;
     const uint32_t window = pick_window((count + stride - 1u) / stride, max(1u, sc.n_lights));
     if (blockIdx.x == 0 && threadIdx.x == 0) wb.counters[rt::WF_SHADOW_WINDOW] = window;
     uint32_t id_next = blockIdx.x * blockDim.x + threadIdx.x < count ? queue[blockIdx.x * blockDim.x + threadIdx.x] : WF_SENTINEL;
@@ -821,6 +834,7 @@
         V3 point = v3(0, 0, 0), normal = point;
         uint32_t material_id = 0;
         DevMaterial m = {};
+        uint32_t map_occluded = 0;
         if (have) {
             uint4 h = wb.hit[id];
             asm volatile("" : "+v"(h.x), "+v"(h.y), "+v"(h.z), "+v"(h.w));
@@ -835,7 +849,18 @@
                     wf_end_path(wb, wf_origin(wb, id), radiance);
                 } else {
                     vertex = true;
+                    const V3 o = point + normal * EXT_EPS;
+                    float map_key = 0.0f, map_k = 0.0f;
+                    if (map_lights) map_k = grid_map_fetch(s_mgrids[0], o, map_key);
                     m = load_material(sc, material_id);
+                    if (map_lights) {
+                        asm volatile("" : "+v"(map_k));
+                        uint32_t rest = map_lights;
+                        if (map_key > map_k) map_occluded |= rest & (0u - rest);
+                        rest &= rest - 1u;
+                        for (uint32_t k = 1; rest; k++, rest &= rest - 1u)
+                            if (grid_map_occluded(s_mgrids[k], o)) map_occluded |= rest & (0u - rest);
+                    }
                     wb.vtx[2 * (size_t)id] = make_float4(point.x, point.y, point.z, __uint_as_float(material_id));
                     if (!shadows) wb.vtx[2 * (size_t)id + 1] = make_float4(normal.x, normal.y, normal.z, 0.0f);
                 }
@@ -852,9 +877,10 @@
                     if (needs_shadow_segment(contrib)) mask |= 1u << li;
                 }
             }
-            if (vertex) wb.vtx[2 * (size_t)id + 1] = make_float4(normal.x, normal.y, normal.z, __uint_as_float(mask));
+            if (vertex) wb.vtx[2 * (size_t)id + 1] = make_float4(normal.x, normal.y, normal.z, __uint_as_float(mask & ~map_occluded));
             if (to_grids) {
                 n_shadow += (uint32_t)__popc(mask);
+                n_map += (uint32_t)__popc(mask & map_occluded);
                 continue;
             }
 #if RT_WF_SHADOW_LIGHT_MAJOR
@@ -889,6 +915,10 @@
     window_close(wb.q_shadow, win);
     const unsigned long long ns = wave_sum(n_shadow);
     if ((threadIdx.x & 63u) == 0 && ns) atomicAdd(&wb.totals[rt::WF_TOTAL_SHADOW], ns);
+    if (map_lights && (fr.flags & RT_FLAG_COUNTERS)) {
+        const unsigned long long nm = wave_sum(n_map);
+        if ((threadIdx.x & 63u) == 0 && nm) atomicAdd(&wb.totals[rt::WF_TOTAL_GRID_ANSWERED], nm), atomicAdd(&wb.totals[rt::WF_TOTAL_MAP_ANSWERED], nm);
+    }
 }
 
 __global__ void k_wf_advance(rt::WfBuffers wb) {
diff --git a/include/rt_hip.h b/include/rt_hip.h
--- a/include/rt_hip.h
+++ b/include/rt_hip.h
@@ -233,9 +233,12 @@
 #define RT_DIRECT_AMBIENT 4u
 #define RT_DIRECT_NO_SHADOWS 8u
 #define RT_DIRECT_NO_SHADOW_GRID 16u
+#define RT_DIRECT_SHADOW_MAP 128u
 #define RT_DIRECT_MAX_LIGHTS 32u
 
 int rt_direct_light(rt_ctx* ctx, const rt_surface_point* points, size_t n, const rt_direct_light_params* params, rt_lighting* out);
+
+int rt_debug_shadow_map(rt_ctx* ctx, unsigned long long out[8]);
 
 typedef struct rt_path_params {
     uint32_t samples;
```

Result: no change. 3337, median of 6 (+0.8%).
